# vfmatzkin/ct-unet

Measured on AMD Instinct MI355X. Metric: voxels/sec fwd+bwd, 128^3 fp32 patch, higher is better.
Workload: dtype f32; 1 GPU; UNet() default (1 in, 2 out, i_size 8, 4 blocks), 128^3 patch, batch 1 per GPU, train step = fwd + Dice/CE loss + bwd + grad all-reduce + Adam(amsgrad); patch=128, per_gpu_batch=1, parallelism=dp1, launch=hipgraph

## Files before the change

### ct-unet_amd/csrc/conv3d.hip

```cpp
#include "common.h"
#include "pack.h"
#include "bn_tail.h"
#include "wgrad_reduce.h"

#ifndef CTU_K3S_OCC
#define CTU_K3S_OCC 2
#endif
#ifndef CTU_K3S_ALL
#define CTU_K3S_ALL 1
#endif
#ifndef CTU_WG_OCC
#define CTU_WG_OCC 2
#endif
#ifndef CTU_WG_BLOCKS
#define CTU_WG_BLOCKS 512
#endif

namespace {

typedef float gv2f __attribute__((ext_vector_type(2)));

struct ConvP {
    const float* in;
    const float* in_scale;
// ... 978 lines not shown
__global__ void pack_batch_kernel(PackTable tb) {
    const ctu_pack_job& q = tb.j[blockIdx.y];
    const int idx = blockIdx.x * blockDim.x + threadIdx.x;
    if (q.kind == 1) {
        const int n16 = (q.nout_p + 15) / 16;
        pack_convt_w_elem(idx, q.w, q.wp, q.Ci, q.Co, q.cinv, q.rin_p, n16 <= 1 ? 1 : (n16 <= 2 ? 2 : (n16 <= 4 ? 4 : 8)), q.mode);
    } else if (q.layout == 1) {
        if (q.k == 3) pack_conv_w_pair8_elem<3>(idx, q.w, q.wp, q.Co, q.Ci, q.cinv, q.rin_p / 8, q.mode);
        else pack_conv_w_pair8_elem<5>(idx, q.w, q.wp, q.Co, q.Ci, q.cinv, q.rin_p / 8, q.mode);
    } else if (q.k == 3) {
        pack_conv_w_elem<3>(idx, q.w, q.wp, q.Co, q.Ci, q.cinv, q.rin_p / 8, (q.nout_p + 15) / 16, q.mode);
    } else {
        pack_conv_w_elem<5>(idx, q.w, q.wp, q.Co, q.Ci, q.cinv, q.rin_p / 8, (q.nout_p + 15) / 16, q.mode);
    }
}



template <int KS>
__global__ void pack_conv_w_kernel(const float* __restrict__ w, float* __restrict__ wp, int Co, int Ci,
                                   const int32_t* __restrict__ cinv, int nchunk, int n16, int mode) {
    pack_conv_w_elem<KS>(blockIdx.x * blockDim.x + threadIdx.x, w, wp, Co, Ci, cinv, nchunk, n16, mode);
}

inline void pick_launch(int N, int D, int H, int W, int k, int nout_p, int* nt, int* td, int* th, int* tw) {
    const int n16 = (nout_p + 15) / 16;
    *nt = n16 == 1 ? 1 : (n16 == 2 ? 2 : 4);
    pick_tile(W, td, th, tw);
    auto blocks = [&](int nt_, int td_, int th_, int tw_) {
        return (long)N * ceil_div(D, td_) * ceil_div(H, th_) * ceil_div(W, tw_) * ceil_div(n16, nt_);
    };
    if (*tw == 16 && *nt > 2) *nt = 2;
    while (blocks(*nt, *td, *th, *tw) < 256 && *nt > 1) *nt >>= 1;
    if (blocks(*nt, *td, *th, *tw) < 256 && *tw > 4) { *td = 4; *th = 4; *tw = 4; }
}

struct WgP {
    const float* in;
    const float* in_scale;
    const float* in_shift;
    const float* g;
    float* ws;
    int in_cs, cin_p, in_relu, g_cs, cout_p;
    int N, D, H, W;
    int tiles_d, tiles_h, tiles_w, ntiles;
    int n_ci_t, n_co_t;
    const float* lz_y;
    float* lz_out;
    const float* lz_scale;
    const float* lz_shift;
    const float* lz_coef;
    int lz_cp;
};

template <int KS, int KDS, int TD, int TH, int TW>
__global__ __launch_bounds__(256, CTU_WG_OCC) void conv3d_wgrad_kernel(WgP p) {
    constexpr int PAD = (KS - 1) / 2;
    constexpr int HD = TD + KDS - 1, HH = TH + KS - 1, HW = TW + KS - 1;
    constexpr int HV = HD * HH * HW;
    constexpr int NVOX = TD * TH * TW;
    constexpr int BT = KDS * KS * KS;
    constexpr int KSTEPS = NVOX / 4;
    constexpr int KPW = KSTEPS / 4;
    static_assert(TW % 4 == 0 && KSTEPS % 4 == 0, "tile shape");

    __shared__ __attribute__((aligned(16))) float sA[HV * 16];
    __shared__ __attribute__((aligned(16))) float sG[NVOX * 16];

    const int tid = threadIdx.x, lane = tid & 63, wave = tid >> 6;
    const int i = lane & 15, kq = lane >> 4;
    const int cit = blockIdx.y % p.n_ci_t, cot = blockIdx.y / p.n_ci_t;
    const int kd0 = blockIdx.z * KDS;
    const int ci0 = cit * 16, co0 = cot * 16;

    f32x4 acc[BT];
#pragma unroll
    for (int t = 0; t < BT; ++t) acc[t] = f32x4{0.f, 0.f, 0.f, 0.f};

    const int quad = tid & 3;
    const bool a_ok = (ci0 + quad * 4) < p.cin_p, g_ok = (co0 + quad * 4) < p.cout_p;
    const bool has_xf = p.in_scale != nullptr;
    float4 sc = make_float4(1.f, 1.f, 1.f, 1.f), sh = make_float4(0.f, 0.f, 0.f, 0.f);
    if (has_xf && a_ok) {
        sc = *reinterpret_cast<const float4*>(p.in_scale + ci0 + quad * 4);
        sh = *reinterpret_cast<const float4*>(p.in_shift + ci0 + quad * 4);
    }

    for (int tile = blockIdx.x; tile < p.ntiles; tile += gridDim.x) {
        int bx = tile;
        const int tx = bx % p.tiles_w; bx /= p.tiles_w;
        const int ty = bx % p.tiles_h; bx /= p.tiles_h;
        const int tz = bx % p.tiles_d; bx /= p.tiles_d;
        const int n_img = bx;
        const int d0 = tz * TD, h0 = ty * TH, w0 = tx * TW;
        __syncthreads();
        constexpr int SB = 8;
        const size_t img = (size_t)n_img * p.D * p.H * p.W;
        for (int it0 = tid; it0 < HV * 4; it0 += SB * 256) {
            f32x4 vv[SB];
            unsigned okm = 0;
#pragma unroll
            for (int q = 0; q < SB; ++q) {
                const int it = it0 + q * 256;
                const int v = (it < HV * 4 ? it : it0) >> 2;
                const int pw = v % HW, t2 = v / HW, ph = t2 % HH, pd = t2 / HH;
                const int gd = d0 + pd + kd0 - PAD, gh = h0 + ph - PAD, gw = w0 + pw - PAD;
// ... 56 lines not shown
    for (int t0 = 0; t0 < BT; t0 += RT) {
        __syncthreads();
#pragma unroll
        for (int t = 0; t < BT; ++t)
            if (t >= t0 && t < t0 + RT) {
#pragma unroll
                for (int r = 0; r < 4; ++r) sA[(wave * RT + (t - t0)) * 256 + (kq * 4 + r) * 16 + i] = acc[t][r];
            }
        __syncthreads();
        const int nt = (BT - t0) < RT ? (BT - t0) : RT;
        for (int e = tid; e < nt * 256; e += 256)
            dst[t0 * 256 + e] = (sA[e] + sA[RT * 256 + e]) + (sA[2 * RT * 256 + e] + sA[3 * RT * 256 + e]);
    }
}

template <int KS, int KDS>
__global__ __launch_bounds__(1024) void conv3d_wgrad_reduce_kernel(const float* __restrict__ ws, float* __restrict__ dw,
                                                                  int Co, int Ci, const int32_t* __restrict__ pmap,
                                                                  int cin_p, int n_ci_t, int gx) {
    constexpr int TAPS = KS * KS * KS, BT = KDS * KS * KS;
    __shared__ float red[RPARTS][64];
    const int e = threadIdx.x & 63, part = threadIdx.x >> 6;
    const int el = blockIdx.x * 64 + e;
    const int pz = blockIdx.y;
    float s = 0.f;
    if (el < BT * 256) {
        const float* src = ws + (size_t)pz * gx * (BT * 256) + el;
        for (int k = part; k < gx; k += RPARTS) s += src[(size_t)k * (BT * 256)];
    }
    red[part][e] = s;
    __syncthreads();
    if (part == 0 && el < BT * 256) {
        const float tot = red_total(red, e);
        const int n_pairs = gridDim.y / (TAPS / BT);
        const int z = pz / n_pairs, pair = pz % n_pairs;
        const int cit = pair % n_ci_t, cot = pair / n_ci_t;
        const int tl = el >> 8, i = (el >> 4) & 15, j = el & 15;
        const int cip = cit * 16 + i, co = cot * 16 + j;
        const int ci = (cip < cin_p) ? (pmap ? pmap[cip] : (cip < Ci ? cip : -1)) : -1;
        if (ci >= 0 && co < Co) dw[((size_t)co * Ci + ci) * TAPS + z * BT + tl] = tot;
    }
}

inline bool use_k3s(int k, int W, int cin_p, int cout_p) { return k == 3 && W >= 16 && (CTU_K3S_ALL || cin_p == 8 || cout_p == 8); }

inline int wgrad_gx(int ntiles, int pairs_z) {
    int gx = CTU_WG_BLOCKS / pairs_z;
    if (gx < 1) gx = 1;
    if (gx > ntiles) gx = ntiles;
    return gx;
}


template <int SM, int SN, int UP = 0, bool LZ = false>
__global__ __launch_bounds__(256, CTU_K3S_OCC) void conv3d_wgrad_k3s_kernel(WgP p, int tiles_per_block) {
    static_assert(!UP || (SM == 1 && SN == 1), "the fused up-convolution uses the full 16 x 16 channel tile");
    constexpr int TD = 4, TH = 4, TW = (SM == 2 && SN == 2) ? 16 : 8, HD = 6, HH = 6, HW = TW + 2, HV = HD * HH * HW;
    constexpr int KPR = TW / 4, NKS = TH * KPR;
    constexpr int CM = 16 / SM, CN = 16 / SN;
    constexpr int GW = TW + (SN - 1), GV = TD * TH * GW;
    constexpr int QN = (SM == 2 && SN == 2) ? 1 : ((SM == 1 && SN == 1) ? 3 : 2);
    constexpr int NMF = UP == 2 ? 12 : (UP ? 8 : 9 * QN);
    constexpr int AQ = CM / 4, GQ = CN / 4;
    constexpr int AITEMS = HV * AQ, AITER = (AITEMS + 255) / 256;
    constexpr int GITEMS = GV * GQ, GITER = (GITEMS + 255) / 256;

    constexpr int SAF = AITER * 256 * 4, SGF = GITER * 256 * 4;
    static_assert(SAF >= HV * CM && SGF >= GV * CN, "stage size");
    __shared__ __attribute__((aligned(16))) float sA[2 * SAF];
    __shared__ __attribute__((aligned(16))) float sG[2 * SGF];

    const int tid = threadIdx.x, lane = tid & 63, wave = tid >> 6;
    const int i = lane & 15, kq = lane >> 4;
    const int cig = blockIdx.y % p.n_ci_t, cog = UP ? (blockIdx.y / p.n_ci_t) % p.n_co_t : blockIdx.y / p.n_ci_t;
    const int par = UP ? blockIdx.y / (p.n_ci_t * p.n_co_t) : 0;
    const int pz = UP == 2 ? (par >> 1) & 1 : (par >> 2) & 1, py = UP == 2 ? par & 1 : (par >> 1) & 1, px = UP == 2 ? 0 : par & 1;
    const int gH = UP ? 2 * p.H : p.H, gW = UP ? 2 * p.W : p.W, gs = UP ? 2 : 1;
    const int ci0 = cig * CM, co0 = cog * CN;
    const bool has_xf = p.in_scale != nullptr;

    f32x4 acc[NMF];
#pragma unroll
    for (int t = 0; t < NMF; ++t) acc[t] = f32x4{0.f, 0.f, 0.f, 0.f};

    const int aq = tid % AQ, gq = tid % GQ;
    const bool a_ok = (ci0 + aq * 4) < p.cin_p, g_ok = (co0 + gq * 4) < p.cout_p;
    float4 sc = make_float4(1.f, 1.f, 1.f, 1.f), sh = make_float4(0.f, 0.f, 0.f, 0.f);
    if (has_xf && a_ok) {
        sc = *reinterpret_cast<const float4*>(p.in_scale + ci0 + aq * 4);
        sh = *reinterpret_cast<const float4*>(p.in_shift + ci0 + aq * 4);
    }
    const int xf_relu = has_xf ? p.in_relu : 0;
    const int boff = (SN == 2) ? ((i < 8) ? i : i - 16) : i;

    int tile = blockIdx.x * tiles_per_block;
    const int tile_end = min(p.ntiles, tile + tiles_per_block);
    float4 va[AITER], vg[GITER];
    float4 vy[LZ ? GITER : 1];
    float4 l_sc = make_float4(0.f, 0.f, 0.f, 0.f), l_sh = l_sc, l_k0 = l_sc, l_A = l_sc, l_B = l_sc;
    if constexpr (LZ) {
        const int lzc = (co0 + ((UP && !g_ok) ? 0 : gq * 4)) % p.lz_cp;
        l_sc = *reinterpret_cast<const float4*>(p.lz_scale + lzc);
        l_sh = *reinterpret_cast<const float4*>(p.lz_shift + lzc);
        l_k0 = *reinterpret_cast<const float4*>(p.lz_coef + lzc);
        l_A = *reinterpret_cast<const float4*>(p.lz_coef + 3 * p.lz_cp + lzc);
        l_B = *reinterpret_cast<const float4*>(p.lz_coef + 4 * p.lz_cp + lzc);
    }
    const long long lz_ydelta = LZ ? reinterpret_cast<const char*>(p.lz_y) - reinterpret_cast<const char*>(p.g) : 0;
    const long long lz_odelta = LZ ? reinterpret_cast<const char*>(p.lz_out) - reinterpret_cast<const char*>(p.g) : 0;

    unsigned aoff[AITER], goff[GITER];
    constexpr int FPW = 5;
    unsigned fw[(AITER + FPW - 1) / FPW], gw0 = 0;
#pragma unroll
    for (int q = 0; q < (AITER + FPW - 1) / FPW; ++q) fw[q] = 0;
#pragma unroll
    for (int it = 0; it < AITER; ++it) {
        const int e = tid + it * 256, v = (e < AITEMS) ? e / AQ : 0;
        const int pw = v % HW, t2 = v / HW, ph = t2 % HH, pd = t2 / HH;
        aoff[it] = (unsigned)(((pd * p.H + ph) * p.W + pw) * p.in_cs + ci0 + aq * 4) * 4u;
        const unsigned face = (pd == 0 ? 1u : 0u) | (pd == HD - 1 ? 2u : 0u) | (ph == 0 ? 4u : 0u) | (ph == HH - 1 ? 8u : 0u) |
                              (pw == 0 ? 16u : 0u) | (pw == HW - 1 ? 32u : 0u);
        fw[it / FPW] |= face << (6 * (it % FPW));
    }
#pragma unroll
    for (int it = 0; it < GITER; ++it) {
        const int e = tid + it * 256, v = (e < GITEMS) ? e / GQ : 0;
        const int tw = v % GW, th = (v / GW) % TH, td = v / (GW * TH);
        goff[it] = (unsigned)(((gs * td * gH + gs * th) * gW + gs * tw) * p.g_cs + co0 + gq * 4) * 4u;
        if (SN == 2 && tw == 0) gw0 |= 1u << it;
    }
    const unsigned safe_a = (unsigned)(((p.H + 1) * p.W + 1) * p.in_cs + ci0 + ((UP && !a_ok) ? 0 : aq * 4)) * 4u;
    const unsigned safe_g = (unsigned)((SN - 1) * p.g_cs + co0 + ((UP && !g_ok) ? 0 : gq * 4)) * 4u;
    const bool ch_full = UP || (ci0 + CM <= p.cin_p && co0 + CN <= p.cout_p);

    struct Box { int tx, ty, tz, n; };
    Box box;
    {
        int t = tile;
        box.tx = t % p.tiles_w; t /= p.tiles_w;
        box.ty = t % p.tiles_h; t /= p.tiles_h;
        box.tz = t % p.tiles_d; box.n = t / p.tiles_d;
    }
    auto box_next = [&](Box b) {
        if (++b.tx == p.tiles_w) { b.tx = 0; if (++b.ty == p.tiles_h) { b.ty = 0; if (++b.tz == p.tiles_d) { b.tz = 0; ++b.n; } } }
        return b;
    };

    unsigned amask = 0, gmask = 0;
    const char* pf_abase = nullptr;
    const char* pf_gbase = nullptr;
    unsigned pf_bface = 0;
    auto prep = [&](Box b) -> bool {
        const int d0 = b.tz * TD, h0 = b.ty * TH, w0 = b.tx * TW;
        const long long org = (((long long)b.n * p.D + d0) * p.H + h0) * p.W + w0;
        pf_abase = reinterpret_cast<const char*>(p.in + (org - ((long long)p.H * p.W + p.W + 1)) * p.in_cs);
        if (UP) {
            const long long gorg = (((long long)b.n * 2 * p.D + 2 * d0 + pz) * gH + 2 * h0 + py) * gW + 2 * w0 + px;
            pf_gbase = reinterpret_cast<const char*>(p.g + gorg * p.g_cs);
        } else {
            pf_gbase = reinterpret_cast<const char*>(p.g + (org - (SN - 1)) * p.g_cs);
        }
        pf_bface = (d0 == 0 ? 1u : 0u) | (d0 + TD == p.D ? 2u : 0u) | (h0 == 0 ? 4u : 0u) | (h0 + TH == p.H ? 8u : 0u) |
                   (w0 == 0 ? 16u : 0u) | (w0 + TW == p.W ? 32u : 0u);
        amask = 0; gmask = 0;
        return ch_full && d0 + TD <= p.D && h0 + TH <= p.H && w0 + TW <= p.W;
    };
    auto fetch_a = [&](int it) {
        const bool ok = (fw[it / FPW] & (pf_bface << (6 * (it % FPW)))) == 0u && (!UP || a_ok);
        va[it] = *reinterpret_cast<const float4*>(pf_abase + (ok ? aoff[it] : safe_a));
        amask |= ok ? (1u << it) : 0u;
    };
    auto fetch_g = [&](int it) {
        const bool ok = !((pf_bface & 16u) && ((gw0 >> it) & 1u)) && (!UP || g_ok);
        const unsigned off = ok ? goff[it] : safe_g;
        vg[it] = *reinterpret_cast<const float4*>(pf_gbase + off);
        if constexpr (LZ) vy[it] = *reinterpret_cast<const float4*>(pf_gbase + lz_ydelta + off);
        gmask |= ok ? (1u << it) : 0u;
    };
    auto load_ragged = [&](Box b) {
        const int d0 = b.tz * TD, h0 = b.ty * TH, w0 = b.tx * TW;
#pragma unroll
        for (int it = 0; it < AITER; ++it) {
            const int e = tid + it * 256, v = e / AQ;
            const int pw = v % HW, t2 = v / HW, ph = t2 % HH, pd = t2 / HH;
            const int gd = d0 + pd - 1, gh = h0 + ph - 1, gw = w0 + pw - 1;
            const bool ok = e < AITEMS && a_ok && (unsigned)gd < (unsigned)p.D && (unsigned)gh < (unsigned)p.H &&
                            (unsigned)gw < (unsigned)p.W;
            float4 val = make_float4(0.f, 0.f, 0.f, 0.f);
            if (ok) {
                val = *reinterpret_cast<const float4*>(pf_abase + aoff[it]);
                amask |= 1u << it;
            }
            va[it] = val;
        }
#pragma unroll
        for (int it = 0; it < GITER; ++it) {
            const int e = tid + it * 256, v = e / GQ;
            const int tw = v % GW, th = (v / GW) % TH, td = v / (GW * TH);
            const int gd = d0 + td, gh = h0 + th, gw = w0 + tw - (SN - 1);
            const bool ok = e < GITEMS && g_ok && gd < p.D && gh < p.H && (unsigned)gw < (unsigned)p.W;
            float4 val = make_float4(0.f, 0.f, 0.f, 0.f);
            if (ok) {
                val = *reinterpret_cast<const float4*>(pf_gbase + goff[it]);
                gmask |= 1u << it;
            }
            vg[it] = val;
        }
    };
// ... 850 lines not shown
                                         int in_relu, const float* ga, int g_cs, int cout_p, const float* y,
                                         const float* bn_scale, const float* bn_shift, const float* coef, float* gy_out,
                                         float* dw, int Co, int Ci, const int32_t* cinv, float* ws, int N, int D, int H, int W,
                                         int k, ctu_wgrad_job* job, void* stream) {
    CTU_REQUIRE(job, "conv3d_wgrad_bn_slabs: null job");
    return conv3d_wgrad_bn_impl(in, in_cs, cin_p, in_scale, in_shift, in_relu, ga, g_cs, cout_p, y, bn_scale, bn_shift, coef,
                                gy_out, dw, Co, Ci, cinv, ws, N, D, H, W, k, job, stream);
}

static int conv3d_wgrad_impl(const float* in, int in_cs, int cin_p, const float* in_scale, const float* in_shift,
                             int in_relu, const float* gout, int g_cs, int cout_p, float* dw, float* dbias, int Co,
                             int Ci, const int32_t* cinv, float* ws, int N, int D, int H, int W, int k, const LazyBn* lz,
                             ctu_wgrad_job* job, void* stream) {
    CTU_REQUIRE(k == 3 || k == 5, "conv3d_wgrad: k=%d unsupported (3 or 5)", k);
    CTU_REQUIRE(in && gout && dw && ws, "conv3d_wgrad: null pointer");
    CTU_REQUIRE(cin_p % 8 == 0 && cout_p % 8 == 0 && cin_p > 0 && cout_p > 0, "conv3d_wgrad: padded channels");
    CTU_REQUIRE(in_cs >= cin_p && in_cs % 4 == 0 && g_cs >= cout_p && g_cs % 4 == 0, "conv3d_wgrad: bad stride");
    CTU_REQUIRE(Co <= cout_p && Co > 0 && Ci > 0 && cin_p <= 256, "conv3d_wgrad: Co/Ci");
    CTU_REQUIRE(((uintptr_t)in & 15) == 0 && ((uintptr_t)gout & 15) == 0, "conv3d_wgrad: 16-byte alignment");
    hipStream_t st = (hipStream_t)stream;
    WgP p;
    p.in = in; p.in_scale = in_scale; p.in_shift = in_shift; p.g = gout; p.ws = ws;
    p.in_cs = in_cs; p.cin_p = cin_p; p.in_relu = in_relu; p.g_cs = g_cs; p.cout_p = cout_p;
    p.N = N; p.D = D; p.H = H; p.W = W;
    p.lz_y = nullptr; p.lz_out = nullptr; p.lz_scale = nullptr; p.lz_shift = nullptr; p.lz_coef = nullptr; p.lz_cp = 0;
    if (lz) { p.lz_y = lz->y; p.lz_out = lz->out; p.lz_scale = lz->scale; p.lz_shift = lz->shift; p.lz_coef = lz->coef; p.lz_cp = lz->cp; }
    const WgPlan r = wgrad_plan(N, D, H, W, k, cin_p, cout_p);
    p.tiles_d = r.tiles_d; p.tiles_h = r.tiles_h; p.tiles_w = r.tiles_w;
    p.ntiles = r.ntiles; p.n_ci_t = r.n_ci_g; p.n_co_t = r.n_co_t;
    int rc;
    if (job) *job = ctu_wgrad_job{};
    if (dbias) job = nullptr;
    if (r.kind == WG_K3S) {
        if (r.sm == 2 && r.sn == 2) rc = launch_wgrad_k3s<2, 2>(p, r, dw, Co, Ci, cinv, st, job);
        else if (r.sn == 2) rc = launch_wgrad_k3s<1, 2>(p, r, dw, Co, Ci, cinv, st, job);
        else if (r.sm == 2) rc = launch_wgrad_k3s<2, 1>(p, r, dw, Co, Ci, cinv, st, job);
        else rc = launch_wgrad_k3s<1, 1>(p, r, dw, Co, Ci, cinv, st, job);
    } else if (r.kind == WG_K5S) {
        CTU_REQUIRE((int64_t)((4 + 2 * 2) * H + 8) * W * in_cs * 4 < (int64_t)1 << 31, "conv3d_wgrad: volume too large for 32-bit offsets");
        if (r.sm == 2 && r.sn == 2) rc = launch_wgrad_k5s<2, 2>(p, r, dw, Co, Ci, cinv, st);
        else if (r.sn == 2) rc = launch_wgrad_k5s<1, 2>(p, r, dw, Co, Ci, cinv, st);
        else rc = launch_wgrad_k5s<2, 1>(p, r, dw, Co, Ci, cinv, st);
    } else rc = (k == 3) ? launch_wgrad<3, 3>(p, r, dw, Co, Ci, cinv, st) : launch_wgrad<5, 1>(p, r, dw, Co, Ci, cinv, st);
    if (rc != CTU_OK) return rc;
    if (dbias) return ctu_channel_sum(gout, g_cs, cout_p, (int64_t)N * D * H * W, ws, dbias, Co, stream);
    return CTU_OK;
}

extern "C" size_t ctu_upconv_fused_wgrad_ws_floats(int N, int D, int H, int W, int cin_p, int nout_p) {
    const size_t na = upwg_plan(N, D, H, W, cin_p, nout_p, false).slabs, nb = upwg_plan(N, D, H, W, cin_p, nout_p, true).slabs;
    return na > nb ? na : nb;
}

static int upconv_fused_wgrad_impl(const float* in, int in_cs, int cin_p, const float* in_scale, const float* in_shift,
                                   int in_relu, const float* gout, int g_cs, int nout_p, float* dweff, float* ws,
                                   int N, int D, int H, int W, const LazyBn* lz, void* stream);

extern "C" int ctu_upconv_fused_wgrad(const float* in, int in_cs, int cin_p, const float* in_scale, const float* in_shift,
                                      int in_relu, const float* gout, int g_cs, int nout_p, float* dweff, float* ws,
                                      int N, int D, int H, int W, void* stream) {
    return upconv_fused_wgrad_impl(in, in_cs, cin_p, in_scale, in_shift, in_relu, gout, g_cs, nout_p, dweff, ws, N, D, H, W,
                                   nullptr, stream);
}

extern "C" int ctu_upconv_fused_wgrad_bn_supported(int N, int D, int H, int W, int cin_p, int nout_p) {
    return (N > 0 && D % 4 == 0 && H % 4 == 0 && W % 8 == 0 && cin_p % 16 == 0 && nout_p % 8 == 0) ? 1 : 0;
}

extern "C" int ctu_upconv_fused_wgrad_bn(const float* in, int in_cs, int cin_p, const float* in_scale, const float* in_shift,
                                         int in_relu, const float* ga, int g_cs, int nout_p, const float* y,
                                         const float* bn_scale, const float* bn_shift, const float* coef, float* gy_out,
                                         float* dweff, float* ws, int N, int D, int H, int W, void* stream) {
    CTU_REQUIRE(y && bn_scale && bn_shift && coef && gy_out, "upconv_fused_wgrad_bn: null pointer");
    CTU_REQUIRE(ctu_upconv_fused_wgrad_bn_supported(N, D, H, W, cin_p, nout_p), "upconv_fused_wgrad_bn: geometry not supported");
    CTU_REQUIRE(((uintptr_t)y & 15) == 0 && ((uintptr_t)gy_out & 15) == 0 && gy_out != ga, "upconv_fused_wgrad_bn: y / gy_out alignment, gy_out must not alias ga");
    const LazyBn lz = {y, bn_scale, bn_shift, coef, gy_out, nout_p};
    return upconv_fused_wgrad_impl(in, in_cs, cin_p, in_scale, in_shift, in_relu, ga, g_cs, nout_p, dweff, ws, N, D, H, W, &lz, stream);
}

static int upconv_fused_wgrad_impl(const float* in, int in_cs, int cin_p, const float* in_scale, const float* in_shift,
                                   int in_relu, const float* gout, int g_cs, int nout_p, float* dweff, float* ws,
                                   int N, int D, int H, int W, const LazyBn* lz, void* stream) {
    CTU_REQUIRE(in && gout && dweff && ws, "upconv_fused_wgrad: null pointer");
    CTU_REQUIRE(cin_p % 8 == 0 && nout_p % 8 == 0 && cin_p > 0 && nout_p > 0 && nout_p <= 64, "upconv_fused_wgrad: padded channels");
    CTU_REQUIRE(in_cs >= cin_p && in_cs % 4 == 0 && g_cs >= nout_p && g_cs % 4 == 0, "upconv_fused_wgrad: bad stride");
    CTU_REQUIRE(((uintptr_t)in & 15) == 0 && ((uintptr_t)gout & 15) == 0, "upconv_fused_wgrad: 16-byte alignment");
    CTU_REQUIRE((in_scale == nullptr) == (in_shift == nullptr), "upconv_fused_wgrad: scale/shift must come together");
    CTU_REQUIRE((int64_t)(2 * H * W + 2 * W + 2) * in_cs * 4 < (int64_t)1 << 31 && (int64_t)(8 * 2 * H + 8) * 2 * W * g_cs * 4 < (int64_t)1 << 31,
                "upconv_fused_wgrad: volume too large for 32-bit offsets");
    hipStream_t st = (hipStream_t)stream;
    const bool pw = nout_p == 8 && g_cs == 8;
    const UpWgPlan g = upwg_plan(N, D, H, W, cin_p, nout_p, pw);
    WgP p;
    p.in = in; p.in_scale = in_scale; p.in_shift = in_shift; p.g = gout; p.ws = ws;
    p.in_cs = in_cs; p.cin_p = cin_p; p.in_relu = in_relu; p.g_cs = g_cs; p.cout_p = nout_p;
    p.N = N; p.D = D; p.H = H; p.W = W;
    p.tiles_d = ceil_div(D, 4); p.tiles_h = ceil_div(H, 4); p.tiles_w = ceil_div(W, 8);
    p.ntiles = g.ntiles; p.n_ci_t = g.n_ci_g; p.n_co_t = g.n_co_g;
    p.lz_y = nullptr; p.lz_out = nullptr; p.lz_scale = nullptr; p.lz_shift = nullptr; p.lz_coef = nullptr; p.lz_cp = 0;
    if (lz) { p.lz_y = lz->y; p.lz_out = lz->out; p.lz_scale = lz->scale; p.lz_shift = lz->shift; p.lz_coef = lz->coef; p.lz_cp = lz->cp; }
    if (pw) {
        p.cout_p = 16;
        if (lz) conv3d_wgrad_k3s_kernel<1, 1, 2, true><<<dim3(g.grid.gx, g.pairs), 256, 0, st>>>(p, g.grid.tpb);
        else conv3d_wgrad_k3s_kernel<1, 1, 2><<<dim3(g.grid.gx, g.pairs), 256, 0, st>>>(p, g.grid.tpb);
        CTU_CHECK_LAUNCH("upconv_fused_wgrad(pw)");
        upconv_wgrad_reduce_pw_kernel<<<dim3(12 * 256 / 64, g.pairs), 64 * RPARTS, 0, st>>>(ws, dweff, cin_p, g.n_ci_g, g.grid.gx);
        CTU_CHECK_LAUNCH("upconv_fused_wgrad_reduce(pw)");
        return CTU_OK;
    }
    if (lz) conv3d_wgrad_k3s_kernel<1, 1, 1, true><<<dim3(g.grid.gx, g.pairs), 256, 0, st>>>(p, g.grid.tpb);
    else conv3d_wgrad_k3s_kernel<1, 1, 1><<<dim3(g.grid.gx, g.pairs), 256, 0, st>>>(p, g.grid.tpb);
    CTU_CHECK_LAUNCH("upconv_fused_wgrad");
    upconv_wgrad_reduce_kernel<<<dim3(8 * 256 / 64, g.pairs), 64 * RPARTS, 0, st>>>(ws, dweff, cin_p, nout_p, g.n_ci_g, g.n_co_g, g.grid.gx);
    CTU_CHECK_LAUNCH("upconv_fused_wgrad_reduce");
    return CTU_OK;
}
```

### ct-unet_amd/csrc/upconv_fused.hip

```cpp
#include <type_traits>
#include "common.h"
#include "bn_tail.h"
#include "channel_sum.h"

namespace {

typedef float v2f __attribute__((ext_vector_type(2)));

struct UpP {
    const float* in;
    const float* in_scale;
    const float* in_shift;
    const float* wp;
    const float* beff;
    float* out;
    float* stats;
    int in_cs, rin_p, in_relu, out_cs, nout_p;
    int N, D, H, W;
    int tiles_d, tiles_h, tiles_w;
    ctu_bn_tail tail;
};

template <int PB, int NTP, bool PW = false>
__global__ __launch_bounds__(256, 2) void upconv_fused_fwd_kernel(UpP p, int ntiles, int tiles_per_block) {
    static_assert(PW ? (PB == 4 && NTP == 1) : ((PB * NTP == 8 || (PB == 4 && NTP == 1)) && (PB == 8 || PB == 4 || PB == 2)), "tile-parities per block");
    constexpr int NTW = PW ? 3 : 2, TAPS = 4 * NTW;
    constexpr int MT = 4, TD = 4, TH = 4, TW = 16;
    constexpr int HD = TD + 2, HH = TH + 2, HW = TW + 2, HV = HD * HH * HW;
    constexpr int NTHR = 256;
    constexpr int NTPT = NTP;
    constexpr int WFL = PB * TAPS * NTP * 128;
    constexpr int AITEMS = HV * 2, AITER = (AITEMS + NTHR - 1) / NTHR;
    constexpr int WITER = (WFL / 4 + NTHR - 1) / NTHR;
    constexpr int VS2 = 6;
    static_assert(WFL / 4 % NTHR == 0, "weight staging covers the stage exactly");

    __shared__ __attribute__((aligned(16))) v2f sA2[HV * VS2];
    __shared__ __attribute__((aligned(16))) v2f sW2[WFL / 2];
    typedef const volatile __attribute__((address_space(3))) v2f* lds_v2f_ptr;
    __shared__ float sRed[4 * NTP * 16 * 2];

    const int tid = threadIdx.x, lane = tid & 63, wave = tid >> 6;
    const int m = lane & 15, kq = lane >> 4;
    const int by = blockIdx.y;
    const int nchunk = p.rin_p >> 3;
    const int half = tid & 1;
    const bool has_xf = p.in_scale != nullptr;
    const int pd0 = PW ? 0 : ((by * PB) >> 2) & 1, ph0 = PW ? 0 : ((by * PB) >> 1) & 1;

    lds_v2f_ptr vA = (lds_v2f_ptr)sA2 + (((wave + pd0) * HH + ph0) * HW + m) * VS2 + kq;
    lds_v2f_ptr vW = (lds_v2f_ptr)sW2 + (kq * 16 + m);

    unsigned hoff[AITER];
    constexpr int FPW = 5, NFW = (AITER + FPW - 1) / FPW;
    unsigned fw[NFW];
#pragma unroll
    for (int q = 0; q < NFW; ++q) fw[q] = 0;
#pragma unroll
    for (int it = 0; it < AITER; ++it) {
        const int i = tid + it * NTHR;
        const int v = (i < AITEMS) ? (i >> 1) : 0;
        const int pw = v % HW, t2 = v / HW, ph = t2 % HH, pd = t2 / HH;
        hoff[it] = (unsigned)(((pd * p.H + ph) * p.W + pw) * p.in_cs + half * 4) * 4u;
        const unsigned face = (pd == 0 ? 1u : 0u) | (pd == HD - 1 ? 2u : 0u) | (ph == 0 ? 4u : 0u) | (ph == HH - 1 ? 8u : 0u) |
                              (pw == 0 ? 16u : 0u) | (pw == HW - 1 ? 32u : 0u);
        fw[it / FPW] |= face << (6 * (it % FPW));
    }
    const unsigned safe_off = (unsigned)(((p.H + 1) * p.W + 1) * p.in_cs + half * 4) * 4u;

    f32x4 acc[PB][MT][NTP];
    float s1[NTP][4], s2[NTP][4];
#pragma unroll
    for (int nt = 0; nt < NTP; ++nt) {
#pragma unroll
        for (int pi = 0; pi < PB; ++pi)
#pragma unroll
            for (int mt = 0; mt < MT; ++mt) acc[pi][mt][nt] = f32x4{0.f, 0.f, 0.f, 0.f};
#pragma unroll
        for (int r = 0; r < 4; ++r) { s1[nt][r] = 0.f; s2[nt][r] = 0.f; }
    }

    int tile = blockIdx.x * tiles_per_block;
    const int tile_end = min(ntiles, tile + tiles_per_block);
    int c = 0;
    float4 va[AITER];
    typedef typename std::conditional<PW, f32x4, float4>::type wv_t;
    wv_t vw[WITER];
    float4 sc = make_float4(1.f, 1.f, 1.f, 1.f), sh = make_float4(0.f, 0.f, 0.f, 0.f);
    unsigned vmask = 0;

    struct Box { int tx, ty, tz, n; };
    Box box;
    {
        int t = tile;
        box.tx = t % p.tiles_w; t /= p.tiles_w;
        box.ty = t % p.tiles_h; t /= p.tiles_h;
        box.tz = t % p.tiles_d; box.n = t / p.tiles_d;
    }
    auto box_next = [&](Box b) {
        if (++b.tx == p.tiles_w) { b.tx = 0; if (++b.ty == p.tiles_h) { b.ty = 0; if (++b.tz == p.tiles_d) { b.tz = 0; ++b.n; } } }
        return b;
    };
    bool a_interior = false;
    auto load_a = [&](Box b, int cc) {
        const int d0 = b.tz * TD, h0 = b.ty * TH, w0 = b.tx * TW;
        if (has_xf) {
            sc = *reinterpret_cast<const float4*>(p.in_scale + cc * 8 + half * 4);
            sh = *reinterpret_cast<const float4*>(p.in_shift + cc * 8 + half * 4);
        }
        const long long org = (((long long)b.n * p.D + d0) * p.H + h0) * p.W + w0 - ((long long)p.H * p.W + p.W + 1);
        const char* base = reinterpret_cast<const char*>(p.in + org * p.in_cs + cc * 8);
        a_interior = d0 >= 1 && h0 >= 1 && w0 >= 1 && d0 + TD < p.D && h0 + TH < p.H && w0 + TW < p.W;
        if (a_interior) {
#pragma unroll
            for (int it = 0; it < AITER; ++it) {
                if ((it + 1) * NTHR <= AITEMS || tid + it * NTHR < AITEMS)
                    va[it] = *reinterpret_cast<const float4*>(base + hoff[it]);
                else
                    va[it] = make_float4(0.f, 0.f, 0.f, 0.f);
            }
            return;
        }
        vmask = 0;
        if (d0 + TD <= p.D && h0 + TH <= p.H && w0 + TW <= p.W) {
            const unsigned bface = (d0 == 0 ? 1u : 0u) | (d0 + TD == p.D ? 2u : 0u) | (h0 == 0 ? 4u : 0u) |
                                   (h0 + TH == p.H ? 8u : 0u) | (w0 == 0 ? 16u : 0u) | (w0 + TW == p.W ? 32u : 0u);
#pragma unroll
            for (int it = 0; it < AITER; ++it) {
                const bool ok = (fw[it / FPW] & (bface << (6 * (it % FPW)))) == 0u;
                va[it] = *reinterpret_cast<const float4*>(base + (ok ? hoff[it] : safe_off));
                vmask |= ok ? (1u << it) : 0u;
            }
            return;
        }
#pragma unroll
        for (int it = 0; it < AITER; ++it) {
            const int i = tid + it * NTHR, v = i >> 1;
            const int pw = v % HW, t2 = v / HW, ph = t2 % HH, pd = t2 / HH;
            const int gd = d0 + pd - 1, gh = h0 + ph - 1, gw = w0 + pw - 1;
            const bool ok = i < AITEMS && (unsigned)gd < (unsigned)p.D && (unsigned)gh < (unsigned)p.H && (unsigned)gw < (unsigned)p.W;
            float4 val = make_float4(0.f, 0.f, 0.f, 0.f);
            if (ok) {
                val = *reinterpret_cast<const float4*>(base + hoff[it]);
                vmask |= 1u << it;
            }
            va[it] = val;
        }
    };
    auto load_w = [&](int cc) {
        const char* wsrc = reinterpret_cast<const char*>(PW ? p.wp + (size_t)cc * 4 * TAPS * 128
                                                            : p.wp + ((size_t)cc * 8 + (size_t)by * PB) * 8 * NTPT * 128);
#pragma unroll
        for (int it = 0; it < WITER; ++it) vw[it] = *reinterpret_cast<const wv_t*>(wsrc + (unsigned)(tid + it * NTHR) * 16u);
    };
    if (tile >= tile_end) return;
    load_a(box, 0);
    load_w(0);

    while (true) {
        CTU_SETPRIO(CTU_PRIO_STAGE);
        __syncthreads();
        {
            auto put = [&](int it, float4 val) {
                const int i = tid + it * NTHR;
// ... 102 lines not shown
                            *reinterpret_cast<float4*>(p.out + fv * p.out_cs + co) = o;
                            s1[nt][0] += o.x; s1[nt][1] += o.y; s1[nt][2] += o.z; s1[nt][3] += o.w;
                            s2[nt][0] += o.x * o.x; s2[nt][1] += o.y * o.y; s2[nt][2] += o.z * o.z; s2[nt][3] += o.w * o.w;
                        }
                        acc[pi][mt][nt] = f32x4{0.f, 0.f, 0.f, 0.f};
                    }
                }
            }
        }
        if (!has_next) break;
        tile = ntile; c = nc; box = nbox;
    }
    if (p.stats) {
        __syncthreads();
#pragma unroll
        for (int nt = 0; nt < NTP; ++nt)
#pragma unroll
            for (int r = 0; r < 4; ++r) {
                float a1 = s1[nt][r], a2 = s2[nt][r];
#pragma unroll
                for (int o = 1; o < 16; o <<= 1) { a1 += __shfl_xor(a1, o); a2 += __shfl_xor(a2, o); }
                if (PW) { a1 += __shfl_xor(a1, 32); a2 += __shfl_xor(a2, 32); }
                const int ch = PW ? (kq & 1) * 4 + r : nt * 16 + kq * 4 + r;
                if (m == 0 && (!PW || kq < 2)) {
                    sRed[(wave * NTP * 16 + ch) * 2 + 0] = a1;
                    sRed[(wave * NTP * 16 + ch) * 2 + 1] = a2;
                }
            }
        __syncthreads();
        float* row = p.stats + ((size_t)blockIdx.y * gridDim.x + blockIdx.x) * 2 * p.nout_p;
        for (int ch = tid; ch < p.nout_p; ch += NTHR) {
            float a1 = 0.f, a2 = 0.f;
#pragma unroll
            for (int w = 0; w < 4; ++w) {
                a1 += sRed[(w * NTP * 16 + ch) * 2 + 0];
                a2 += sRed[(w * NTP * 16 + ch) * 2 + 1];
            }
            st_row(p.tail.counter != nullptr, row + ch, a1);
            st_row(p.tail.counter != nullptr, row + p.nout_p + ch, a2);
        }
        if (p.tail.counter) bn_fwd_tail(p.tail, p.stats, gridDim.x * gridDim.y, p.nout_p, gridDim.x * gridDim.y);
    }
}

struct UpDP {
    const float* g;
    const float* wp;
    float* out;
    int g_cs, nout_p, out_cs, cin_p;
    int N, D, H, W;
    int tiles_d, tiles_h, tiles_w, n16;
};

template <int NT>
__global__ __launch_bounds__(256, 2) void upconv_fused_bwd_data_kernel(UpDP p, int ntiles, int tiles_per_block) {
    constexpr int MT = 4, TD = 4, TH = 4, TW = 16;
    constexpr int HD = TD + 2, HH = TH + 2, HW = TW + 2, HV = HD * HH * HW;
    constexpr int NTHR = 256;
    constexpr int WFL = 8 * NT * 128;
    constexpr int AITEMS = HV * 2, AITER = (AITEMS + NTHR - 1) / NTHR;
    constexpr int WITER = (WFL / 4 + NTHR - 1) / NTHR;
    constexpr int VS2 = 6;
    static_assert(WFL / 4 % NTHR == 0, "weight staging covers the stage exactly");

    __shared__ __attribute__((aligned(16))) v2f sA2[HV * VS2];
    __shared__ __attribute__((aligned(16))) v2f sW2[WFL / 2];
    typedef const volatile __attribute__((address_space(3))) v2f* lds_v2f_ptr;

    const int tid = threadIdx.x, lane = tid & 63, wave = tid >> 6;
    const int m = lane & 15, kq = lane >> 4;
    const int by = blockIdx.y;
    const int qc = p.nout_p >> 3;
    const int nchunk = 8 * qc;
    const int half = tid & 1;
    const int Hf = 2 * p.H, Wf = 2 * p.W;

    lds_v2f_ptr vA0 = (lds_v2f_ptr)sA2 + ((wave * HH) * HW + m) * VS2 + kq;
    lds_v2f_ptr vW = (lds_v2f_ptr)sW2 + (kq * 16 + m);

    unsigned hoff[AITER];
    constexpr int FPW = 5, NFW = (AITER + FPW - 1) / FPW;
    unsigned fw[NFW];
#pragma unroll
    for (int q = 0; q < NFW; ++q) fw[q] = 0;
#pragma unroll
    for (int it = 0; it < AITER; ++it) {
        const int i = tid + it * NTHR;
        const int v = (i < AITEMS) ? (i >> 1) : 0;
        const int pw = v % HW, t2 = v / HW, ph = t2 % HH, pd = t2 / HH;
        hoff[it] = (unsigned)(((2 * pd * Hf + 2 * ph) * Wf + 2 * pw) * p.g_cs + half * 4) * 4u;
        const unsigned face = (pd == 0 ? 1u : 0u) | (pd == HD - 1 ? 2u : 0u) | (ph == 0 ? 4u : 0u) | (ph == HH - 1 ? 8u : 0u) |
                              (pw == 0 ? 16u : 0u) | (pw == HW - 1 ? 32u : 0u);
        fw[it / FPW] |= face << (6 * (it % FPW));
    }
    const unsigned safe_off = (unsigned)(((2 * Hf + 2) * Wf + 2) * p.g_cs + half * 4) * 4u;

    f32x4 acc[MT][NT];
#pragma unroll
    for (int nt = 0; nt < NT; ++nt)
#pragma unroll
        for (int mt = 0; mt < MT; ++mt) acc[mt][nt] = f32x4{0.f, 0.f, 0.f, 0.f};

    int tile = blockIdx.x * tiles_per_block;
    const int tile_end = min(ntiles, tile + tiles_per_block);
    if (tile >= tile_end) return;
    int c = 0;
    float4 va[AITER], vw[WITER];
    unsigned vmask = 0;
// ... 99 lines not shown
        if (nc == nchunk) { nc = 0; ntile = tile + 1; nbox = box_next(box); }
        const bool has_next = ntile < tile_end;
        if (has_next) {
            load_a(nbox, nc);
            load_w(nc);
        }
        CTU_SETPRIO(0);
        {
            v2f ar[2][5], br[2][2][NT];
            auto load_group = [&](int g, v2f (&aa)[5], v2f (&bb)[2][NT]) {
                const int ez = (g >> 1) & 1, ex = g & 1;
#pragma unroll
                for (int r = 0; r < 5; ++r) aa[r] = vA[((ez * HH + r) * HW + ex) * VS2];
#pragma unroll
                for (int ey = 0; ey < 2; ++ey)
#pragma unroll
                    for (int nt = 0; nt < NT; ++nt) bb[ey][nt] = vW[(((ez * 2 + ey) * 2 + ex) * NT + nt) * 64];
            };
            load_group(0, ar[0], br[0]);
#if CTU_PIN_FWD
            __builtin_amdgcn_sched_barrier(0);
#endif
#pragma unroll
            for (int g = 0; g < 4; ++g) {
                if (g + 1 < 4) load_group(g + 1, ar[(g + 1) & 1], br[(g + 1) & 1]);
                v2f (&aa)[5] = ar[g & 1];
                v2f (&bb)[2][NT] = br[g & 1];
#pragma unroll
                for (int ey = 0; ey < 2; ++ey) {
#pragma unroll
                    for (int nt = 0; nt < NT; ++nt)
#pragma unroll
                        for (int mt = 0; mt < MT; ++mt)
                            acc[mt][nt] = __builtin_amdgcn_mfma_f32_16x16x4f32(bb[ey][nt].x, aa[mt + ey].x, acc[mt][nt], 0, 0, 0);
#pragma unroll
                    for (int nt = 0; nt < NT; ++nt)
#pragma unroll
                        for (int mt = 0; mt < MT; ++mt)
                            acc[mt][nt] = __builtin_amdgcn_mfma_f32_16x16x4f32(bb[ey][nt].y, aa[mt + ey].y, acc[mt][nt], 0, 0, 0);
                }
#if CTU_PIN_FWD
#pragma unroll
                for (int q = 0; q < 4 * MT * NT; ++q) {
                    __builtin_amdgcn_sched_group_barrier(0x008, 1, 0);
                    if (g + 1 < 4 && q < 5 + 2 * NT) __builtin_amdgcn_sched_group_barrier(0x100, 1, 0);
                }
#endif
            }
        }
        CTU_SETPRIO(CTU_PRIO_STAGE);
        if (c == nchunk - 1) {
            const int d0 = box.tz * TD, h0 = box.ty * TH, w0 = box.tx * TW;
            const int gw = w0 + m;
            float* obase = p.out + ((((size_t)box.n * p.D + d0 + wave) * p.H + h0) * p.W + gw) * p.out_cs;
            const int orow = p.W * p.out_cs;
#pragma unroll
            for (int nt = 0; nt < NT; ++nt) {
                const int co = (by * NT + nt) * 16 + kq * 4;
#pragma unroll
                for (int mt = 0; mt < MT; ++mt) {
                    if (co < p.cin_p && d0 + wave < p.D && h0 + mt < p.H && gw < p.W) {
                        float4 o;
                        o.x = acc[mt][nt][0]; o.y = acc[mt][nt][1]; o.z = acc[mt][nt][2]; o.w = acc[mt][nt][3];
                        *reinterpret_cast<float4*>(obase + mt * orow + co) = o;
                    }
                    acc[mt][nt] = f32x4{0.f, 0.f, 0.f, 0.f};
                }
            }
        }
        if (!has_next) break;
        tile = ntile; c = nc; box = nbox;
    }
}

__device__ __forceinline__ float upconv_pack_bwd_value(const float* __restrict__ wp, int idx, int cin_p, int nout_p) {
    const int n16 = (cin_p + 15) >> 4, qc = nout_p >> 3, ntpt = (nout_p + 15) >> 4;
    int r = idx;
    const int j = r & 1; r >>= 1;
    const int n = r & 15; r >>= 4;
    const int kq = r & 3; r >>= 2;
    const int nt = r % n16; r /= n16;
    const int e = r & 7; r >>= 3;
    const int q = r % qc;
    const int par = r / qc;
    const int pos = nt * 16 + n, co = q * 8 + kq * 2 + j;
    float v = 0.f;
    if (pos < cin_p) {
        const int cf = pos >> 3, kqf = (pos & 7) >> 1, jf = pos & 1;
        v = wp[((((size_t)cf * 8 + par) * 8 + (e ^ 7)) * ntpt + (co >> 4)) * 128 + kqf * 32 + (co & 15) * 2 + jf];
    }
    return v;
}

__device__ __forceinline__ int axis_pairs(int pbit, int jbit, int (&t)[2], int (&a)[2]) {
    if (pbit == 0) {
        if (jbit == 0) { t[0] = 0; a[0] = 1; return 1; }
        t[0] = 1; a[0] = 0; t[1] = 2; a[1] = 1; return 2;
    }
    if (jbit == 0) { t[0] = 0; a[0] = 0; t[1] = 1; a[1] = 1; return 2; }
    t[0] = 2; a[0] = 0; return 1;
}

__global__ void upconv_transpose_kernel(const float* __restrict__ wt, const float* __restrict__ w3, float* __restrict__ wtt,
                                        float* __restrict__ w3t, int C, int Co, int nout_p) {
    const int idx = blockIdx.x * blockDim.x + threadIdx.x;
    const int n3 = 27 * C * nout_p, nt = 8 * C * C;
    if (idx < n3) {
        const int co = idx % nout_p, cm = (idx / nout_p) % C, t = idx / (nout_p * C);
        w3t[idx] = co < Co ? w3[((size_t)co * C + cm) * 27 + t] : 0.f;
    } else if (idx < n3 + nt) {
        const int k = idx - n3;
        const int cm = k % C, ci = (k / C) % C, a = k / (C * C);
        wtt[k] = wt[((size_t)ci * C + cm) * 8 + a];
    }
}

constexpr int WS_WAVES = 8, WS_BLOCK = WS_WAVES * 64;
// ... 306 lines not shown
}

extern "C" int ctu_upconv_fused_supported(int k, int D, int H, int W, int cin_p, int nout_p) {
    return k == 3 && W >= 16 && D >= 1 && H >= 1 && cin_p % 8 == 0 && cin_p >= 8 && nout_p % 8 == 0 && nout_p >= 8 && nout_p <= 64;
}

static size_t up_std_packed(int cin_p, int nout_p) { return (size_t)(cin_p / 8) * 8 * 8 * ceil_div(nout_p, 16) * 128; }

extern "C" size_t ctu_upconv_fused_packed_floats(int cin_p, int nout_p) {
    return up_std_packed(cin_p, nout_p) + (nout_p == 8 ? (size_t)(cin_p / 8) * 4 * 12 * 128 : 0);
}

extern "C" int ctu_upconv_fused_num_blocks(int N, int D, int H, int W, int nout_p) {
    const UpPlan r = up_plan(N, D, H, W, nout_p, 0);
    return r.grid.gx * r.ny;
}

extern "C" size_t ctu_upconv_fused_pack_ws_floats(int C, int nout_p) { return (size_t)27 * C * nout_p + (size_t)8 * C * C; }

static int upconv_pack_gather(const float* wp, int cin_p, int nout_p, float* wpw, float* wpd, hipStream_t st) {
    const int npw = wpw ? (cin_p / 8) * 4 * 12 * 128 : 0;
    const int nwpd = wpd ? (int)ctu_upconv_fused_bwd_packed_floats(cin_p, nout_p) : 0;
    if (npw + nwpd == 0) return CTU_OK;
    upconv_pack_gather_kernel<<<ceil_div(npw + nwpd, 256), 256, 0, st>>>(wp, wpw, npw, wpd, nwpd, cin_p, nout_p);
    CTU_CHECK_LAUNCH("upconv_fused_pack_gather");
    return CTU_OK;
}

extern "C" int ctu_upconv_fused_pack_all(const float* wt, const float* bt, const float* w3, int C, int Co, const int32_t* cinv,
                                         int cin_p, int nout_p, float* wp, float* beff, float* ws, float* wpd, void* stream) {
    CTU_REQUIRE(wt && bt && w3 && wp && beff && ws, "upconv_fused_pack: null pointer");
    CTU_REQUIRE(C > 0 && Co > 0 && Co <= nout_p && cin_p % 8 == 0 && nout_p % 8 == 0 && (cinv || C <= cin_p),
                "upconv_fused_pack: C=%d Co=%d cin_p=%d nout_p=%d", C, Co, cin_p, nout_p);
    hipStream_t st = (hipStream_t)stream;
    const int ntpt = ceil_div(nout_p, 16);
    CTU_REQUIRE(((uintptr_t)ws & 15) == 0, "upconv_fused_pack: ws must be 16-byte aligned");
    float* w3t = ws;
    float* wtt = ws + (size_t)27 * C * nout_p;
    const int ntr = 27 * C * nout_p + 8 * C * C;
    upconv_transpose_kernel<<<ceil_div(ntr, 256), 256, 0, st>>>(wt, w3, wtt, w3t, C, Co, nout_p);
    CTU_CHECK_LAUNCH("upconv_fused_transpose");
    const int quads = (cin_p / 8) * 8 * 8 * 8 * ntpt * 4;
    upconv_pack_beff_kernel<<<nout_p / BEFF_CO + ceil_div(quads, 8), WS_BLOCK, 0, st>>>(wtt, w3t, wp, C, nout_p, cinv, cin_p / 8,
                                                                                         ntpt, bt, beff);
    CTU_CHECK_LAUNCH("upconv_fused_pack");
    return upconv_pack_gather(wp, cin_p, nout_p, nout_p == 8 ? wp + up_std_packed(cin_p, nout_p) : nullptr, wpd, st);
}

extern "C" int ctu_upconv_fused_pack(const float* wt, const float* bt, const float* w3, int C, int Co, const int32_t* cinv,
                                     int cin_p, int nout_p, float* wp, float* beff, float* ws, void* stream) {
    return ctu_upconv_fused_pack_all(wt, bt, w3, C, Co, cinv, cin_p, nout_p, wp, beff, ws, nullptr, stream);
}

extern "C" int ctu_upconv_fused_fwd(const float* in, int in_cs, int cin_p, const float* in_scale, const float* in_shift,
                                    int in_relu, const float* wp, const float* beff, float* out, int out_cs, int nout_p,
                                    float* stats, int N, int D, int H, int W, const ctu_bn_tail* tail, void* stream) {
    CTU_REQUIRE(in && wp && beff && out, "upconv_fused_fwd: null pointer");
    CTU_REQUIRE(ctu_upconv_fused_supported(3, D, H, W, cin_p, nout_p), "upconv_fused_fwd: unsupported geometry (W=%d cin_p=%d nout_p=%d)",
                W, cin_p, nout_p);
    CTU_REQUIRE(in_cs >= cin_p && in_cs % 4 == 0 && out_cs >= nout_p && out_cs % 4 == 0, "upconv_fused_fwd: bad stride");
    CTU_REQUIRE((in_scale == nullptr) == (in_shift == nullptr), "upconv_fused_fwd: scale/shift must come together");
    CTU_REQUIRE(((uintptr_t)in & 15) == 0 && ((uintptr_t)out & 15) == 0 && ((uintptr_t)wp & 15) == 0 && ((uintptr_t)beff & 15) == 0,
                "upconv_fused_fwd: 16-byte alignment");
    CTU_REQUIRE((int64_t)N * D * H * W * 8 < (int64_t)1 << 31 && (int64_t)(2 * H * W + 2 * W + 2) * in_cs * 4 < (int64_t)1 << 31,
                "upconv_fused_fwd: volume too large for 32-bit offsets");
    UpP p;
    p.in = in; p.in_scale = in_scale; p.in_shift = in_shift; p.wp = wp; p.beff = beff; p.out = out; p.stats = stats;
    CTU_REQUIRE(!tail || (stats && tail->counter && tail->gamma && tail->beta && tail->scale && tail->shift && tail->mean &&
                          tail->invstd && tail->C > 0 && tail->C <= nout_p && tail->count > 0),
                "upconv_fused_fwd: incomplete BatchNorm tail");
    p.tail = tail_or_off(tail);
    p.in_cs = in_cs; p.rin_p = cin_p; p.in_relu = in_relu; p.out_cs = out_cs; p.nout_p = nout_p;
    p.N = N; p.D = D; p.H = H; p.W = W;
    const UpPlan r = up_plan(N, D, H, W, nout_p, 0);
    p.tiles_d = r.tiles_d; p.tiles_h = r.tiles_h; p.tiles_w = r.tiles_w;
    const int ny = r.ny, gx = r.grid.gx, tpb = r.grid.tpb, ntiles = r.ntiles;
    hipStream_t st = (hipStream_t)stream;
    if (nout_p == 16 && ny == 2) {
        upconv_fused_fwd_kernel<4, 1><<<dim3(gx, 2), 256, 0, st>>>(p, ntiles, tpb);
    } else if (nout_p == 8) {
        p.wp = wp + up_std_packed(cin_p, nout_p);
        upconv_fused_fwd_kernel<4, 1, true><<<dim3(gx, 1), 256, 0, st>>>(p, ntiles, tpb);
    } else if (ny == 1) upconv_fused_fwd_kernel<8, 1><<<dim3(gx, 1), 256, 0, st>>>(p, ntiles, tpb);
    else if (ny == 2) upconv_fused_fwd_kernel<4, 2><<<dim3(gx, 2), 256, 0, st>>>(p, ntiles, tpb);
    else upconv_fused_fwd_kernel<2, 4><<<dim3(gx, 4), 256, 0, st>>>(p, ntiles, tpb);
    CTU_CHECK_LAUNCH("upconv_fused_fwd");
    return CTU_OK;
}

extern "C" int ctu_channel_sum_num_blocks(int64_t nvox);

extern "C" size_t ctu_upconv_fused_project_ws_floats(int nout_p, int64_t fine_nvox) {
    return (size_t)27 * FS_SPLIT * nout_p + (size_t)27 * nout_p + nout_p + (size_t)ctu_channel_sum_num_blocks(fine_nvox) * nout_p;
}

static int upconv_project_impl(int dtype, const float* dweff, const void* gout, int g_cs, int nout_p, int N, int D, int H, int W,
                               const float* bt, const float* pack_ws, const int32_t* imap, int C, int Co, int cin_p,
                               float* dwt, float* dbt, float* dw3, float* ws, void* stream) {
    CTU_REQUIRE(dweff && gout && bt && pack_ws && dwt && dbt && dw3 && ws, "upconv_fused_project: null pointer");
    CTU_REQUIRE(nout_p == 8 || nout_p == 16 || nout_p == 32 || nout_p == 64, "upconv_fused_project: nout_p=%d", nout_p);
    CTU_REQUIRE(C > 0 && Co > 0 && Co <= nout_p && g_cs >= nout_p && g_cs % 4 == 0, "upconv_fused_project: bad channels");
    CTU_REQUIRE(((uintptr_t)dweff & 15) == 0 && ((uintptr_t)pack_ws & 15) == 0, "upconv_fused_project: dweff / pack_ws must be 16-byte aligned");
    hipStream_t st = (hipStream_t)stream;
    float* tpart = ws;
    float* V = ws + (size_t)27 * FS_SPLIT * nout_p;
    float* tall = V + (size_t)27 * nout_p;
    float* csp = tall + nout_p;
    const int64_t fvox = (int64_t)N * 8 * D * H * W;
    const int nb = ctu_channel_sum_num_blocks(fvox);
    const int nsum = nb + 26 * FS_SPLIT;
    if (dtype == 0) {
        upconv_sums_kernel<float><<<nsum, 256, 0, st>>>((const float*)gout, g_cs, nout_p, N, 2 * D, 2 * H, 2 * W, fvox, csp, nb, tpart);
    } else {
        CTU_DISPATCH_LP(dtype, upconv_sums_kernel<T><<<nsum, 256, 0, st>>>((const T*)gout, g_cs, nout_p, N, 2 * D, 2 * H, 2 * W, fvox, csp, nb, tpart));
    }
    CTU_CHECK_LAUNCH("upconv_sums");
    upconv_tall_v_kernel<<<nout_p, 256, 0, st>>>(csp, nb, tpart, nout_p, tall, V);
    CTU_CHECK_LAUNCH("upconv_tall_v");
    const float* w3t = pack_ws;
    const float* wtt = pack_ws + (size_t)27 * C * nout_p;
    const int nb1 = ceil_div((C * C * 8 + C) * 8, WS_BLOCK);
    const int nb2 = ceil_div(((Co + 3) / 4) * C * 27, 8);
    upconv_project_kernel<<<nb1 + nb2, WS_BLOCK, 0, st>>>(dweff, V, wtt, w3t, bt, imap, C, Co, cin_p, nout_p, nb1, dwt, dw3, dbt);
    CTU_CHECK_LAUNCH("upconv_project");
    return CTU_OK;
}

extern "C" int ctu_upconv_fused_project(const float* dweff, const float* gout, int g_cs, int nout_p, int N, int D, int H, int W,
                                        const float* bt, const float* pack_ws, const int32_t* imap, int C, int Co, int cin_p,
                                        float* dwt, float* dbt, float* dw3, float* ws, void* stream) {
    return upconv_project_impl(0, dweff, gout, g_cs, nout_p, N, D, H, W, bt, pack_ws, imap, C, Co, cin_p, dwt, dbt, dw3, ws, stream);
}
extern "C" int ctu_lp_upconv_fused_project(int dtype, const float* dweff, const void* gout, int g_cs, int nout_p, int N, int D, int H,
                                           int W, const float* bt, const float* pack_ws, const int32_t* imap, int C, int Co, int cin_p,
                                           float* dwt, float* dbt, float* dw3, float* ws, void* stream) {
    CTU_REQUIRE(dtype == CTU_BF16 || dtype == CTU_F16, "lp_upconv_fused_project: dtype %d", dtype);
    return upconv_project_impl(dtype, dweff, gout, g_cs, nout_p, N, D, H, W, bt, pack_ws, imap, C, Co, cin_p, dwt, dbt, dw3, ws, stream);
}

extern "C" size_t ctu_upconv_fused_bwd_packed_floats(int cin_p, int nout_p) {
    return (size_t)8 * (nout_p / 8) * 8 * ceil_div(cin_p, 16) * 128;
}

extern "C" int ctu_upconv_fused_pack_bwd(const float* wp, int cin_p, int nout_p, float* wpd, void* stream) {
    CTU_REQUIRE(wp && wpd && cin_p % 8 == 0 && nout_p % 8 == 0, "upconv_fused_pack_bwd: bad argument");
    return upconv_pack_gather(wp, cin_p, nout_p, nullptr, wpd, (hipStream_t)stream);
}

extern "C" int ctu_upconv_fused_bwd_data(const float* gout, int g_cs, int nout_p, const float* wpd, float* gin, int gin_cs,
                                         int cin_p, int N, int D, int H, int W, void* stream) {
    CTU_REQUIRE(gout && wpd && gin, "upconv_fused_bwd_data: null pointer");
    CTU_REQUIRE(ctu_upconv_fused_supported(3, D, H, W, cin_p, nout_p), "upconv_fused_bwd_data: unsupported geometry");
    CTU_REQUIRE(g_cs >= nout_p && g_cs % 4 == 0 && gin_cs >= cin_p && gin_cs % 4 == 0, "upconv_fused_bwd_data: bad stride");
    CTU_REQUIRE(((uintptr_t)gout & 15) == 0 && ((uintptr_t)gin & 15) == 0 && ((uintptr_t)wpd & 15) == 0, "upconv_fused_bwd_data: alignment");
    CTU_REQUIRE((int64_t)(12 * 2 * H + 12) * 2 * W * g_cs * 4 + 64 < (int64_t)1 << 31, "upconv_fused_bwd_data: volume too large for 32-bit offsets");
    UpDP p;
    p.g = gout; p.wp = wpd; p.out = gin; p.g_cs = g_cs; p.nout_p = nout_p; p.out_cs = gin_cs; p.cin_p = cin_p;
    p.N = N; p.D = D; p.H = H; p.W = W;
    p.n16 = ceil_div(cin_p, 16);
    const UpPlan r = up_plan(N, D, H, W, nout_p, p.n16);
    p.tiles_d = r.tiles_d; p.tiles_h = r.tiles_h; p.tiles_w = r.tiles_w;
    const int NT = r.nt, ny = r.ny, gx = r.grid.gx, tpb = r.grid.tpb, ntiles = r.ntiles;
    hipStream_t st = (hipStream_t)stream;
    if (NT == 4) upconv_fused_bwd_data_kernel<4><<<dim3(gx, ny), 256, 0, st>>>(p, ntiles, tpb);
    else if (NT == 2) upconv_fused_bwd_data_kernel<2><<<dim3(gx, ny), 256, 0, st>>>(p, ntiles, tpb);
    else upconv_fused_bwd_data_kernel<1><<<dim3(gx, ny), 256, 0, st>>>(p, ntiles, tpb);
    CTU_CHECK_LAUNCH("upconv_fused_bwd_data");
    return CTU_OK;
}
```

### ct-unet_amd/ctunet_amd/_lib.py

```python
from __future__ import annotations

import ctypes as C
import os

import torch

_HERE = os.path.dirname(os.path.abspath(__file__))
LIB_PATH = os.environ.get("CTUNET_HIP_LIB") or os.path.join(_HERE, "libctunet_hip.so")

P = C.c_void_p
I = C.c_int
L = C.c_int64
F = C.c_float
D = C.c_double
Z = C.c_size_t
U = C.c_uint64

class PackJob(C.Structure):
    _fields_ = [("w", C.c_void_p), ("wp", C.c_void_p), ("cinv", C.c_void_p), ("kind", C.c_int), ("Co", C.c_int),
                ("Ci", C.c_int), ("k", C.c_int), ("rin_p", C.c_int), ("nout_p", C.c_int), ("mode", C.c_int),
                ("layout", C.c_int)]


class BnTail(C.Structure):
# ... 54 lines not shown
    "ctu_bn_bwd_num_blocks": (I, [L]),
    "ctu_bn_relu_bwd_reduce": (I, [P, I, P, I, I, P, P, P, P, L, P, P, P]),
    "ctu_bn_bwd_finalize": (I, [P, I, I, I, D, P, P, P, P, P, P, P, P, F, F, P, P]),
    "ctu_bn_relu_bwd_apply": (I, [P, I, P, I, I, P, P, P, P, P, L, P]),
    "ctu_conv3d_wgrad_slabs": (I, [P, I, I, P, P, I, P, I, I, P, P, I, I, P, P, I, I, I, I, I, P, P]),
    "ctu_conv3d_wgrad_bn_slabs": (I, [P, I, I, P, P, I, P, I, I, P, P, P, P, P, P, I, I, P, P, I, I, I, I, I, P, P]),
    "ctu_conv3d_first_wgrad_slabs": (I, [P, I, P, I, P, I, P, I, I, I, I, P, P]),
    "ctu_conv3d_first_wgrad_bn_slabs": (I, [P, I, P, I, P, P, P, P, P, P, I, P, I, I, I, I, P, P]),
    "ctu_convt2_wgrad_slabs": (I, [P, I, I, P, P, I, P, I, I, P, P, I, I, P, P, I, I, I, I, P, P]),
    "ctu_bn_bwd_finalize_jobs": (I, [P, I, I, I, D, P, P, P, P, P, P, P, P, F, F, P, P, I, P]),
    "ctu_wgrad_reduce_jobs": (I, [P, I, P]),
    "ctu_maxpool2_fwd": (I, [P, I, I, P, P, I, P, I, I, I, I, I, P]),
    "ctu_maxpool2_bwd": (I, [P, I, I, P, P, I, P, I, P, I, I, I, I, I, I, P]),
    "ctu_maxpool2_bwd_bn_num_blocks": (I, [I, I, I, I, I]),
    "ctu_maxpool2_bwd_bn": (I, [P, I, I, P, P, P, P, P, I, P, I, I, I, I, I, I, P, P, P]),
    "ctu_convt_packed_floats": (Z, [I, I]),
    "ctu_pack_convt_weight": (I, [P, P, I, I, P, I, I, I, P]),
    "ctu_convt2_fwd": (I, [P, I, I, P, P, I, P, P, I, P, I, I, I, I, I, I, P]),
    "ctu_convt2_bwd_data": (I, [P, I, I, P, P, I, I, I, I, I, I, P]),
    "ctu_convt2_wgrad_ws_floats": (Z, [I, I, I, I, I, I]),
    "ctu_convt2_wgrad": (I, [P, I, I, P, P, I, P, I, I, P, P, I, I, P, P, I, I, I, I, P]),
    "ctu_convt2_plan": (C.c_char_p, [I, I, I, I, I, I, I, P]),
    "ctu_convt2_wgrad_plan": (C.c_char_p, [I, I, I, I, I, I, P]),
    "ctu_head_fwd": (I, [P, I, I, P, P, I, P, P, P, I, I, I, I, P, P, I, L, P]),
    "ctu_head_bwd_ws_floats": (Z, [I, L, I, I]),
    "ctu_head_bwd": (I, [P, I, I, P, P, I, P, P, P, I, I, I, I, P, P, P, I, P, P, P, I, L, P]),
    "ctu_head_bwd_num_blocks": (I, [I, L]),
    "ctu_head_bwd_bn": (I, [P, I, I, P, P, I, P, P, P, I, I, I, I, P, P, P, I, P, P, P, I, L, P, P, I, P, P, P]),
    "ctu_head_fwd_seg2": (I, [P, I, P, I, I, P, P, I, P, P, P, I, I, I, I, P, P, I, L, P]),
    "ctu_head_bwd_bn_seg2": (I, [P, I, P, I, I, P, P, I, P, P, P, I, I, I, I, P, P, P, I, P, I, P, P, P, I, L, P, P, I, P, P, P]),
    "ctu_loss_ws_floats": (Z, [I, L]),
    "ctu_loss_fwd": (I, [P, P, I, L, F, F, I, P, P, P]),
    "ctu_loss_bwd": (I, [P, P, I, L, F, F, I, P, P, P, P, I, P]),
    "ctu_seg_loss_ws_floats": (Z, [I, L]),
    "ctu_seg_loss_fwd": (I, [P, P, P, I, L, P, P, P, P]),
    "ctu_seg_loss_bwd": (I, [P, P, P, I, L, P, P, P, P, P, P, P, I, P]),
    "ctu_skip_add": (I, [P, I, P, P, I, P, I, P, P, I, P, I, I, L, P]),
    "ctu_upconv_fused_supported": (I, [I, I, I, I, I, I]),
    "ctu_upconv_fused_packed_floats": (Z, [I, I]),
    "ctu_upconv_fused_num_blocks": (I, [I, I, I, I, I]),
    "ctu_upconv_fused_pack_ws_floats": (Z, [I, I]),
    "ctu_upconv_fused_pack": (I, [P, P, P, I, I, P, I, I, P, P, P, P]),
    "ctu_upconv_fused_pack_all": (I, [P, P, P, I, I, P, I, I, P, P, P, P, P]),
    "ctu_upconv_fused_fwd": (I, [P, I, I, P, P, I, P, P, P, I, I, P, I, I, I, I, P, P]),
    "ctu_upconv_fused_wgrad_ws_floats": (Z, [I, I, I, I, I, I]),
    "ctu_upconv_fused_wgrad": (I, [P, I, I, P, P, I, P, I, I, P, P, I, I, I, I, P]),
    "ctu_upconv_fused_wgrad_bn_supported": (I, [I, I, I, I, I, I]),
    "ctu_upconv_fused_wgrad_bn": (I, [P, I, I, P, P, I, P, I, I, P, P, P, P, P, P, P, I, I, I, I, P]),
    "ctu_upconv_fused_project_ws_floats": (Z, [I, L]),
    "ctu_upconv_fused_project": (I, [P, P, I, I, I, I, I, I, P, P, P, I, I, I, P, P, P, P, P]),
    "ctu_upconv_fused_bwd_packed_floats": (Z, [I, I]),
    "ctu_upconv_fused_pack_bwd": (I, [P, I, I, P, P]),
    "ctu_upconv_fused_bwd_data": (I, [P, I, I, P, P, I, I, I, I, I, I, P]),
    "ctu_hard_segm": (I, [P, I, I, L, P, P]),
    "ctu_one_hot": (I, [P, I, I, L, P, P]),
    "ctu_hard_dice_ws_doubles": (Z, [I]),
    "ctu_hard_dice_counts": (I, [P, P, I, I, L, P, P, P]),
    "ctu_hausdorff_ws_bytes": (Z, [I, I, I, I, I]),
    "ctu_hausdorff": (I, [P, P, I, I, I, I, I, P, P, P]),
    "ctu_surface_ws_bytes": (Z, [I, I, I, I, I]),
    "ctu_surface_metrics": (I, [P, I, I, P, I, I, I, I, I, I, I, I, I, P, P, D, P, P, P]),
    "ctu_components_ws_bytes": (Z, [I, I, I, I]),
    "ctu_label_components": (I, [P, I, I, I, I, I, I, P, I, P, P, P, P]),
    "ctu_filter_components": (I, [P, I, I, I, I, I, I, P, I, I, I, P, P, P]),
    "ctu_morphology_ws_bytes": (Z, [I, I, I, I, I]),
    "ctu_binary_morphology": (I, [P, I, I, I, I, I, I, C.c_uint32, I, I, I, L, P, P, P]),
    "ctu_fill_holes": (I, [P, I, I, I, I, I, I, I, L, P, P, P]),
    "ctu_implant_mask": (I, [P, I, P, I, I, I, I, I, C.c_uint32, I, I, I, I, P, P, P]),
    "ctu_distance_ws_bytes": (Z, [I, I, I, I, I, I]),
    "ctu_distance_transform": (I, [P, I, I, I, I, I, I, L, I, I, P, I, P, P, F, P, P]),
    "ctu_thickness_ws_bytes": (Z, [I, I, I, I, I]),
    "ctu_local_thickness": (I, [P, I, I, I, I, I, P, P, P, P]),
    "ctu_thickness_summary_ws_bytes": (Z, [I, L]),
    "ctu_thickness_summary": (I, [P, I, L, F, P, P, P]),
    "ctu_resample": (I, [P, I, I, I, L, I, I, I, I, I, I, P, P, P, P, P]),
    "ctu_affine_resample": (I, [P, I, I, I, L, I, I, I, I, I, I, P, P, P, P, P, D, P, P]),
    "ctu_registration_ws_bytes": (Z, [L]),
    "ctu_registration_init": (I, [P, L, P, P, P]),
    "ctu_registration_accumulate": (I, [P, L, P, I, I, I, P, P, D, P, P]),
    "ctu_registration_update": (I, [L, I, P, P, P, I, P, P]),
    "ctu_similarity_ws_bytes": (Z, [L, L]),
    "ctu_similarity_init": (I, [P, L, P, P, P]),
    "ctu_similarity_accumulate": (I, [I, P, L, P, I, I, I, P, P, P, L, P, I, I, I, P, P, D, P, P]),
    "ctu_similarity_update": (I, [I, L, L, I, P, P, P, I, P, P]),
    "ctu_ffd_ws_bytes": (Z, [P, L]),
    "ctu_ffd_cells": (I, [P, L, P, P, P, P, P, P]),
    "ctu_ffd_init": (I, [P, L, P, D, P, P, P]),
    "ctu_ffd_accumulate": (I, [P, L, P, P, I, I, I, P, P, P, P, P, D, P, P, P, P, L, P, P]),
    "ctu_ffd_update": (I, [L, P, P, P, P, L, I, P, P, I, P, P]),
    "ctu_ffd_transform_points": (I, [P, L, P, P, P, P, P, P, P, P]),
    "ctu_ffd_resample": (I, [P, I, I, I, L, I, I, I, I, I, I, P, P, P, P, P, P, P, P, P, D, P, P]),
    "ctu_mesh_ws_bytes": (Z, [I, I, I]),
    "ctu_mesh_count": (I, [P, I, I, I, I, I, L, F, P, P]),
    "ctu_mesh_emit": (I, [P, I, I, I, I, F, F, P, P, L, L, P, P, P, P]),
    "ctu_mesh_measure": (I, [P, L, P, L, P, P, P, P]),
    "ctu_mesh_adjacency_ws_bytes": (Z, [L, L]),
    "ctu_mesh_adjacency_build": (I, [P, L, L, P, P, P]),
    "ctu_mesh_adjacency_emit": (I, [L, L, L, P, P, P, P]),
    "ctu_mesh_smooth_ws_bytes": (Z, [L]),
    "ctu_mesh_smooth": (I, [P, L, P, P, L, P, I, F, I, F, P, P, P]),
    "ctu_mesh_voxelize_ws_bytes": (Z, [I, I, I]),
    "ctu_mesh_voxelize": (I, [P, L, P, L, I, I, I, P, P, I, P, P, P]),
    "ctu_mesh_grid_ws_bytes": (Z, [L, L]),
    "ctu_mesh_grid_build": (I, [P, L, P, L, F, L, P, P, P]),
    "ctu_mesh_grid_emit": (I, [P, L, L, L, L, P, P, P, P]),
    "ctu_mesh_distance": (I, [P, L, P, P, L, P, I, I, I, P, L, I, I, I, P, P, F, F, P, P, P, P]),
# ... 179 lines not shown
```

### ct-unet_amd/ctunet_amd/engine.py

```python
from __future__ import annotations

import os
from dataclasses import dataclass
from typing import Dict, List, Optional, Tuple

import torch

from . import ops
from .ops import CL, pad8

BN_EPS = 1e-5
FUSE_UP = os.environ.get("CTUNET_FUSE_UP", "1") != "0"
FUSE_UP_MAX_CO = int(os.environ.get("CTUNET_FUSE_UP_MAXCO", "16"))
POOL_BN = os.environ.get("CTUNET_POOL_BN", "1") != "0"
LP_FUSE_UP = os.environ.get("CTUNET_LP_FUSE_UP", "1") != "0"
BN_MOMENTUM = 0.1
LAZY_BN = os.environ.get("CTUNET_LAZY_BN", "1") != "0"
LAZY_BN_LP = os.environ.get("CTUNET_LAZY_BN_LP", "0") != "0"
BN_TAIL = os.environ.get("CTUNET_BN_TAIL", "0") != "0"
DEFER_WGRAD_REDUCE = os.environ.get("CTUNET_DEFER_WGRAD_REDUCE", "1") != "0"
SPLIT_CAT0 = os.environ.get("CTUNET_SPLIT_CAT0", "1") != "0"


def _cat_halves(buf: torch.Tensor, cp: int):
    if buf.dim() == 6:
        return CL(buf[0], 0, cp), CL(buf[1], 0, cp)
    return CL(buf, 0, cp), CL(buf, cp, cp)


@dataclass
class BlockPlan:
    prefix: str
    first: int
    cin: int
    cout: int


@dataclass
class NetPlan:
    k: int
    conv_bias: bool
    in_ch: int
    out_ch: int
    enc: List[BlockPlan]
    center: BlockPlan
    center_live: bool
    dec: List[BlockPlan]
    head: str
    act: int
    head_mode: int
    skip: str = "cat"


@dataclass(slots=True)
class _ConvRec:
    x: Optional[CL]
    y: CL
    vec: torch.Tensor
    stats: Optional[torch.Tensor]
    nblk: int
    conv: str
    bn: str
    cin: int
    cout: int
    imap: Optional[torch.Tensor]
    bias: bool
    first: Optional[torch.Tensor] = None


class _WgradWs:

    def __init__(self, floats: int, device, defer: bool):
        self.jobs = ops.WgradJobs() if defer else None
        self.bufs = [torch.empty(floats, dtype=torch.float32, device=device) for _ in range(2 if defer else 1)]
        self.i = 0

    def take(self) -> torch.Tensor:
        self.i = (self.i + 1) % len(self.bufs)
        ws = self.bufs[self.i]
        if self.jobs is not None:
# ... 89 lines not shown
                continue
            ver = (w._version, w.data_ptr())
            if force or ent[0] != ver:
                jobs.append((kind, w.detach().contiguous(), ent[1], ent[2], rin_p, nout_p, mode, layout))
                self._pack_cache[key] = (ver, ent[1], ent[2])
        ops.pack_batch(jobs, self.dtype)

    def invalidate_packs(self) -> None:
        for key, ent in self._pack_cache.items():
            self._pack_cache[key] = (None,) + tuple(ent[1:])
        for prefix, hit in self._up_cache.items():
            self._up_cache[prefix] = (None,) + tuple(hit[1:])

    def _fwd_tail(self, P, bn: str, c: int, nvox: int, n_upd: int, vec4: torch.Tensor, device):
        counter = self._counter(bn, "fwd", device)
        if counter is None:
            return None
        return ops.make_bn_tail(c, nvox, P[bn + ".weight"], P[bn + ".bias"], P[bn + ".running_mean"], P[bn + ".running_var"],
                                BN_MOMENTUM, BN_EPS, n_upd, vec4, P.get(bn + ".num_batches_tracked") if n_upd else None,
                                counter)

    def _bn_stage(self, P, bn: str, out: CL, vec4: torch.Tensor, nvox: int, c: int, training: bool, n_upd: int, nblk: int,
                  launch, tail_ok: bool = True) -> Tuple[CL, Optional[torch.Tensor]]:
        wb = (P[bn + ".weight"], P[bn + ".bias"], P[bn + ".running_mean"], P[bn + ".running_var"])
        if training:
            stats = torch.empty((nblk, 2, out.cp), dtype=torch.float32, device=out.buf.device)
            tail = self._fwd_tail(P, bn, c, nvox, n_upd, vec4, out.buf.device) if tail_ok else None
            launch(stats, tail)
            if tail is None:
                ops.bn_finalize_into(stats, nblk, c, out.cp, nvox, *wb, BN_MOMENTUM, BN_EPS, n_upd, vec4,
                                     P.get(bn + ".num_batches_tracked") if n_upd else None)
        else:
            stats = None
            launch(None, None)
            ops.bn_eval_affine_into(*wb, BN_EPS, c, out.cp, vec4)
        return out.with_xf(vec4[0], vec4[1], True), stats

    def _conv_bn(self, P, x: CL, conv: str, bn: str, cin: int, cout: int, imap, out: CL, vec4: torch.Tensor,
                 training: bool, n_upd: int, save: bool) -> Tuple[CL, Optional[_ConvRec]]:
        k = self.plan.k
        w = P[conv + ".weight"]
        bias = P.get(conv + ".bias")
        lay = ops.conv_layout(k, out.cp, x.dims[3], self.dtype, x.cp)
        if bias is not None and self.dtype != torch.float32:
            lay = 0
        wp = self._packed(conv, w, "conv", imap, x.cp, out.cp, 0, lay)
        bias_p = None if bias is None else bias.detach()
        nblk = ops.conv_num_blocks(x.dims, out.cp, lay, k, self.dtype, x.cp) if training else 0
        y, stats = self._bn_stage(P, bn, out, vec4, x.nvox, cout, training, n_upd, nblk,
                                  lambda stats, tail: ops.conv3d_fwd(x, wp, bias_p, out, k, stats, (cin, cout), lay, tail))
        rec = _ConvRec(x, out.raw(), vec4, stats, nblk, conv, bn, cin, cout, imap, bias is not None) if save else None
        return y, rec

    def _fuse_up(self, x: CL, nout_p: int) -> bool:
        if not (self.plan.k == 3 and not self.plan.conv_bias and nout_p <= FUSE_UP_MAX_CO and FUSE_UP):
            return False
        if self.dtype == torch.float32:
            return ops.upconv_fused_supported(x.dims, 3, x.cp, nout_p)
        return LP_FUSE_UP and ops.lp_upconv_fused_supported(x.dims, 3, x.cp, nout_p)

    def _upconv_bn(self, P, x: CL, prefix: str, ct: int, cout: int, cinv, out: CL, vec4: torch.Tensor, training: bool,
                   n_upd: int, save: bool) -> Tuple[CL, Optional[_ConvRec]]:
        conv, bn = f"{prefix}.1", f"{prefix}.2"
        wt, bt, w3 = P[f"{prefix}.0.weight"], P[f"{prefix}.0.bias"], P[conv + ".weight"]
        lp = bool(x.lp)
        ver = tuple((t._version, t.data_ptr()) for t in (wt, bt, w3))
        hit = self._up_cache.get(prefix)
        if hit is None or hit[0] != ver or hit[3] != (x.cp, out.cp, self.dtype) or torch.cuda.is_current_stream_capturing():
            same = hit is not None and hit[3] == (x.cp, out.cp, self.dtype)
            if lp:
                wp, beff, pws = ops.upconv_fused_pack(wt, bt, w3, cinv, x.cp, out.cp, (hit[1], hit[2], hit[4]) if same else None)
                wpd = ops.lp_upconv_fused_pack(wp, x.cp, self.dtype, hit[5] if same else None)
            else:
                wp, beff, pws, wpd = ops.upconv_fused_pack_all(wt, bt, w3, cinv, x.cp, out.cp,
                                                               (hit[1], hit[2], hit[4], hit[5]) if same else None)
            self._up_cache[prefix] = (ver, wp, beff, (x.cp, out.cp, self.dtype), pws, wpd)
        else:
            wp, beff, wpd = hit[1], hit[2], hit[5]
        if lp:
            nblk = ops.lp_upconv_fused_num_blocks(x.dims) if training else 0
            launch = lambda stats, tail: ops.lp_upconv_fused_fwd(x, wpd, beff, out, stats, (ct, cout))
        else:
            nblk = ops.upconv_fused_num_blocks(x.dims, out.cp) if training else 0
            launch = lambda stats, tail: ops.upconv_fused_fwd(x, wp, beff, out, stats, (ct, cout), tail)
        y, stats = self._bn_stage(P, bn, out, vec4, 8 * x.nvox, cout, training, n_upd, nblk, launch, tail_ok=not lp)
        rec = _ConvRec(None, out.raw(), vec4, stats, nblk, conv, bn, ct, cout, None, False) if save else None
        return y, rec

    def _first_conv_bn(self, P, x: torch.Tensor, conv: str, bn: str, cin: int, cout: int, out: CL, vec4: torch.Tensor,
                       training: bool, n_upd: int, save: bool):
        w = P[conv + ".weight"].detach()
        bias = P.get(conv + ".bias")
        bias_p = None if bias is None else bias.detach()
        nblk = ops.conv_first_num_blocks(out.dims) if training else 0
        y, stats = self._bn_stage(P, bn, out, vec4, out.nvox, cout, training, n_upd, nblk,
                                  lambda stats, tail: ops.conv_first_fwd(x, w, bias_p, out, stats, tail))
        rec = _ConvRec(None, out.raw(), vec4, stats, nblk, conv, bn, cin, cout, None, bias is not None, x) if save else None
        return y, rec

    def forward(self, P: Dict[str, torch.Tensor], x: torch.Tensor, training: bool, save: bool, chk: bool):
        plan = self.plan
        dev = x.device
        n, cin, d, h, w = x.shape
        nlev = len(plan.enc)
        if cin != plan.in_ch:
            raise RuntimeError(f"ctunet_amd: expected {plan.in_ch} input channels, got {cin}")
        if any(s % (1 << nlev) for s in (d, h, w)):
            raise RuntimeError(f"ctunet_amd: spatial size {(d, h, w)} must be divisible by {1 << nlev}")
        if training and n * (d >> nlev) * (h >> nlev) * (w >> nlev) <= 1:
            raise ValueError("Expected more than 1 value per channel when training (centre block)")
        ctx = {"recs": {}, "levels": [], "training": training, "chk": chk} if save else None
        n_upd = 1 if training else 0
        self.refresh_packs(P)

        x = x.contiguous()
        e0 = plan.enc[0]
        first_direct = plan.conv_bias is False and ops.conv_first_supported(plan.k, cin, pad8(e0.cout), w)
        adt = self.dtype
        cur = None if first_direct else ops.ncdhw_to_cl(x, dtype=adt)
        x_cl = cur
        cat: List[torch.Tensor] = []
        halves = []
        xf: List[torch.Tensor] = []
        pooled: List[CL] = []
        dskip: List[CL] = []
        dd, hh, ww = d, h, w
        recs = {}
        xf_sizes = [8 * pad8(blk.cout) for blk in plan.enc]
        xf_all = torch.zeros(sum(xf_sizes), dtype=torch.float32, device=dev)
        xf_off = 0
        for i, blk in enumerate(plan.enc):
            cp = pad8(blk.cout)
            split = SPLIT_CAT0 and i == 0 and cp <= 16
            cat.append(torch.empty((2, n, dd, hh, ww, cp) if split else (n, dd, hh, ww, 2 * cp), dtype=adt, device=dev))
            halves.append(_cat_halves(cat[i], cp))
            xf.append(xf_all[xf_off:xf_off + 8 * cp].view(4, 2 * cp))
            xf_off += 8 * cp
            t1 = CL(torch.empty((n, dd, hh, ww, cp), dtype=adt, device=dev), 0, cp)
            v1 = torch.empty((4, cp), dtype=torch.float32, device=dev)
            imap = None
            if i == 0 and first_direct:
                a1, recs[(blk.prefix, 1)] = self._first_conv_bn(P, x, f"{blk.prefix}.{blk.first}",
                                                                f"{blk.prefix}.{blk.first + 1}", blk.cin, blk.cout, t1,
                                                                v1, training, n_upd, save)
            else:
                a1, recs[(blk.prefix, 1)] = self._conv_bn(P, cur, f"{blk.prefix}.{blk.first}",
                                                          f"{blk.prefix}.{blk.first + 1}", blk.cin, blk.cout, imap, t1,
                                                          v1, training, n_upd, save)
            a2, recs[(blk.prefix, 2)] = self._conv_bn(P, a1, f"{blk.prefix}.{blk.first + 3}", f"{blk.prefix}.{blk.first + 4}",
                                                      blk.cout, blk.cout, None, halves[i][1], xf[i][:, cp:],
                                                      training, n_upd, save)
            dskip.append(a2)
            dd, hh, ww = dd // 2, hh // 2, ww // 2
            pl = CL(torch.empty((n, dd, hh, ww, cp), dtype=adt, device=dev), 0, cp)
            ops.maxpool_fwd(a2, pl)
            pooled.append(pl)
            cur = pl
        cb = plan.center
        cpc = pad8(cb.cout)
        center_out = None
        if plan.center_live or training:
            live = plan.center_live
            c1 = CL(torch.empty((n, dd, hh, ww, cpc), dtype=adt, device=dev), 0, cpc)
            c2 = CL(torch.empty((n, dd, hh, ww, cpc), dtype=adt, device=dev), 0, cpc)
            v1 = torch.empty((4, cpc), dtype=torch.float32, device=dev)
            v2 = torch.empty((4, cpc), dtype=torch.float32, device=dev)
            a1, r1 = self._conv_bn(P, cur, f"{cb.prefix}.{cb.first}", f"{cb.prefix}.{cb.first + 1}", cb.cin, cb.cout,
                                   None, c1, v1, training, n_upd, save and live)
            a2, r2 = self._conv_bn(P, a1, f"{cb.prefix}.{cb.first + 3}", f"{cb.prefix}.{cb.first + 4}", cb.cout, cb.cout,
                                   None, c2, v2, training, n_upd, save and live)
            if live:
                recs[(cb.prefix, 1)], recs[(cb.prefix, 2)] = r1, r2
                center_out = a2
        cur = center_out if plan.center_live else pooled[-1]
        cur_segs = ((cb.cout if plan.center_live else plan.enc[-1].cout, 0),)
        dec_in: List[CL] = []
        ups: List[CL] = []
        for j, blk in enumerate(plan.dec):
            i = nlev - 1 - j
            cp = pad8(blk.cout)
            dd, hh, ww = dd * 2, hh * 2, ww * 2
            ct = blk.cin
            ctp = pad8(ct)
            imap_t, cinv_t = self._maps(cur_segs, cur.cp, dev)
            wt = P[f"{blk.prefix}.0.weight"]
            dec_in.append(cur)
            t1 = CL(torch.empty((n, dd, hh, ww, cp), dtype=adt, device=dev), 0, cp)
            v1 = torch.empty((4, cp), dtype=torch.float32, device=dev)
            if self._fuse_up(cur, cp):
                ups.append(None)
                a1, recs[(blk.prefix, 1)] = self._upconv_bn(P, cur, blk.prefix, ct, blk.cout, cinv_t, t1, v1, training,
                                                            n_upd, save)
            else:
                up = CL(torch.empty((n, dd, hh, ww, ctp), dtype=adt, device=dev), 0, ctp)
                wpt = self._packed(f"{blk.prefix}.0", wt, "convt", cinv_t, cur.cp, ctp, 0)
                ops.convt_fwd(cur, wpt, P[f"{blk.prefix}.0.bias"].detach(), up)
                ups.append(up)
                a1, recs[(blk.prefix, 1)] = self._conv_bn(P, up, f"{blk.prefix}.1", f"{blk.prefix}.2", ct, blk.cout, None,
                                                          t1, v1, training, n_upd, save)
            a2, recs[(blk.prefix, 2)] = self._conv_bn(P, a1, f"{blk.prefix}.4", f"{blk.prefix}.5", blk.cout, blk.cout, None,
                                                      halves[i][0], xf[i][:, :cp], training, n_upd, save)
            h_dec, h_enc = halves[i]
            if plan.skip == "cat":
                if cat[i].dim() == 6:
                    cur = ops.CL2(h_dec, h_enc, xf[i][0], xf[i][1], True)
                else:
                    cur = CL(cat[i], 0, 2 * cp, xf[i][0], xf[i][1], True)
                cur_segs = ((blk.cout, 0), (blk.cout, cp))
            elif plan.skip == "none":
                cur = h_dec.with_xf(xf[i][0][:cp], xf[i][1][:cp])
                cur_segs = ((blk.cout, 0),)
            else:
                cur = CL(torch.empty((n, dd, hh, ww, cp), dtype=adt, device=dev), 0, cp)
                ops.skip_add(h_dec.with_xf(xf[i][0][:cp], xf[i][1][:cp]), h_enc.with_xf(xf[i][0][cp:], xf[i][1][cp:]), cur)
                cur_segs = ((blk.cout, 0),)
        imap_h, _ = self._maps(cur_segs, cur.cp, dev)
        wl, bl = P[plan.head + ".weight"], P[plan.head + ".bias"]
        w2 = wl.detach().reshape(wl.shape[0], wl.shape[1])
        out0, out1 = ops.head_fwd(cur, w2, bl.detach(), imap_h, plan.act, plan.head_mode)
        if save:
            ctx.update(recs=recs, x_cl=x_cl, cat=cat, xf=xf, pooled=pooled, dskip=dskip, dec_in=dec_in, ups=ups,
                       head_in=cur, imap_h=imap_h, center_out=center_out, dims=(n, d, h, w))
        return out0, out1, ctx

    def _replay(self, P, rec: _ConvRec):
        return ((P[rec.bn + ".running_mean"], P[rec.bn + ".running_var"], BN_MOMENTUM, BN_EPS,
                 P.get(rec.bn + ".num_batches_tracked")) if self._replay_stats else None)

    def _bwd_fin(self, P, rec: _ConvRec, device):
        counter = self._counter(rec.bn, "bwd", device)
        return None if counter is None else (P[rec.bn + ".weight"].detach(), rec.cout, self._replay(P, rec), counter)

    def _gy_like(self, ga: CL) -> CL:
        ent = self._gy_bufs.get(id(ga.buf))
        if ent is None:
            ent = self._gy_bufs[id(ga.buf)] = (ga.buf, torch.empty_like(ga.buf))
        return CL(ent[1], ga.c0, ga.cp)

    def _conv_bn_bwd(self, P, rec: _ConvRec, ga: CL, gin: Optional[CL], grads: Dict[str, torch.Tensor], ws: _WgradWs, part,
                     pre_reduced: Optional[int] = None, finalized=None, up_in: Optional[CL] = None):
        k = self.plan.k
        can = LAZY_BN and ga.cs == rec.y.cs and (not ga.lp or LAZY_BN_LP)
        if up_in is not None:
            lazy = can and (ops.lp_upconv_fused_wgrad_bn_supported(up_in.dims, up_in.cp) if ga.lp else
                            ops.upconv_fused_wgrad_bn_supported(up_in.dims, up_in.cp, ga.cp))
        elif rec.first is not None:
            lazy = can and not rec.bias and not ga.lp
        else:
            lazy = can and not rec.bias and rec.x is not None and ops.conv3d_wgrad_bn_supported(ga.dims, k, rec.x.cp, ga.cp, self.dtype)
        jobs = ws.jobs
        res = ops.bn_relu_bwd(rec.y, ga, rec.vec, P[rec.bn + ".weight"].detach(), rec.cout, part, self._replay(P, rec),
                              pre_reduced, self._counter(rec.bn, "bwd", ga.buf.device), finalized, lazy, jobs)
        grads[rec.bn + ".weight"], grads[rec.bn + ".bias"] = res[0], res[1]
        if up_in is not None:
            return (rec.y, rec.vec, res[2], self._gy_like(ga)) if lazy else None
        if rec.first is not None:
            if lazy:
                gy = self._gy_like(ga)
                grads[rec.conv + ".weight"] = ops.conv_first_wgrad_bn(rec.first, ga, rec.y, rec.vec, res[2], gy, rec.cout,
                                                                      ws.take(), jobs)
                ga = gy
            else:
                grads[rec.conv + ".weight"] = ops.conv_first_wgrad(rec.first, ga, rec.cout, ws.take(), jobs)
            return ops.conv_first_bwd_data(ga, P[rec.conv + ".weight"].detach(), rec.cin) if gin is not None else None
        if lazy:
            gy = self._gy_like(ga)
            grads[rec.conv + ".weight"] = ops.conv3d_wgrad_bn(rec.x, ga, rec.y, rec.vec, res[2], gy, rec.cout, rec.cin, k,
                                                             rec.imap, ws.take(), jobs)
            ga = gy
        elif rec.x is not None:
            dw, dbias = ops.conv3d_wgrad(rec.x, ga, rec.cout, rec.cin, k, rec.imap, ws.take(), rec.bias, jobs)
            grads[rec.conv + ".weight"] = dw
            if rec.bias:
                grads[rec.conv + ".bias"] = dbias
        if gin is not None:
# ... 7 lines not shown
        recs = ctx["recs"]
        n, d, h, w = ctx["dims"]
        dev = g0.device
        nlev = len(plan.enc)
        gs = 1.0
        flag = None
        dyn = self.scaler if self.dtype == torch.float16 else None
        if dyn is not None:
            dyn.prepare(dev, n * d * h * w)
            flag = dyn.found_inf
        elif self.dtype == torch.float16:
            gs = self.loss_scale if self.loss_scale else float(2 ** max(0, (n * d * h * w).bit_length() - 5))
            flag = self.overflow_flag(dev)
            flag.zero_()
        grads: Dict[str, torch.Tensor] = {}
        emitted: set = set()
        self._gy_bufs = {}

        def unscale(tensors):
            if dyn is not None:
                ops.unscale_tensors(tensors, dyn.scale, flag)
            elif gs != 1.0:
                ops.scale_tensors(tensors, 1.0 / gs, flag)

        def emit():
            new = [(nm, g) for nm, g in grads.items() if nm not in emitted and g is not None]
            emitted.update(nm for nm, _ in new)
            if sync is not None or dyn is not None or gs != 1.0:
                ws.flush()
            unscale([g for _, g in new])
            if sync is not None:
                sync.push(new)
        k = plan.k
        ws_n, part_n = 1, 1
        for r in recs.values():
            if r is None:
                continue
            if r.first is not None:
                ws_n = max(ws_n, ops.conv_first_wgrad_ws(r.y.dims, r.cin))
                part_n = max(part_n, ops.bn_bwd_partials_floats(r.y.nvox, r.y.cp))
                continue
            ws_n = max(ws_n, ops.conv3d_wgrad_ws(r.y.dims, k, r.x.cp if r.x is not None else pad8(r.cin), r.y.cp, self.dtype))
            part_n = max(part_n, ops.bn_bwd_partials_floats(r.y.nvox, r.y.cp))
        for x_in, blk in zip(ctx["dec_in"], plan.dec):
            ws_n = max(ws_n, ops.convt_wgrad_ws(x_in.dims, x_in.cp, pad8(blk.cin), self.dtype))
        for dsk in ctx["dskip"]:
            part_n = max(part_n, ops.maxpool_bwd_bn_blocks(dsk.dims, dsk.cp) * 2 * dsk.cp)
        part_n = max(part_n, ops.head_bwd_blocks(ctx["head_in"].dims) * 2 * pad8(plan.dec[-1].cout))
        ws = _WgradWs(ws_n, dev, DEFER_WGRAD_REDUCE and self.dtype == torch.float32 and ops.TIMER is None)
        part = torch.empty(part_n, dtype=torch.float32, device=dev)

        self._replay_stats = bool(ctx["training"] and ctx["chk"])

        cat, head_in = ctx["cat"], ctx["head_in"]
        gcat = [torch.empty_like(c) for c in cat]
        ghalves = [_cat_halves(g, g.shape[-1] // (1 if g.dim() == 6 else 2)) for g in gcat]
        wl, bl = P[plan.head + ".weight"], P[plan.head + ".bias"]
        w2 = wl.detach().reshape(wl.shape[0], wl.shape[1])
        gsd = None if dyn is None else dyn.scale
        def g_skip_target(level: int) -> CL:
            g_dec, g_enc = ghalves[level]
            if plan.skip != "cat":
                return g_dec
            return ops.CL2(g_dec, g_enc) if gcat[level].dim() == 6 else CL(gcat[level], 0, 2 * g_dec.cp)

        def g_skip_fanout(level: int):
            if plan.skip == "add":
                ops.skip_add(ghalves[level][0], None, ghalves[level][1])

        r_last = recs[(plan.dec[-1].prefix, 2)]
        head_rows, head_fin = None, None
        head_lo = head_in.a if isinstance(head_in, ops.CL2) else head_in
        if (POOL_BN and head_in.scale is not None and head_in.relu and head_in.scale.data_ptr() == r_last.vec[0].data_ptr()
                and head_lo.c0 == r_last.y.c0 and head_lo.buf is r_last.y.buf):
            fin = self._bwd_fin(P, r_last, dev)
            res = ops.head_bwd(head_in, w2, bl.detach(), ctx["imap_h"], plan.act, plan.head_mode, g0.contiguous(),
                               None if g1 is None else g1.contiguous(), g_skip_target(0), (r_last.vec, part), fin, gscale=gs,
                               gscale_dev=gsd)
            dwl, dbl, head_rows = res[:3]
            head_fin = res[3] if fin is not None else None
        else:
            dwl, dbl = ops.head_bwd(head_in, w2, bl.detach(), ctx["imap_h"], plan.act, plan.head_mode, g0.contiguous(),
                                    None if g1 is None else g1.contiguous(), g_skip_target(0), gscale=gs,
                                    gscale_dev=gsd)
        g_skip_fanout(0)
        grads[plan.head + ".weight"], grads[plan.head + ".bias"] = dwl.reshape(wl.shape), dbl
        emit()

        g_deep: Optional[CL] = None
        for j in range(nlev - 1, -1, -1):
            blk = plan.dec[j]
            i = nlev - 1 - j
            cp = pad8(blk.cout)
            r1, r2 = recs[(blk.prefix, 1)], recs[(blk.prefix, 2)]
            g_u2 = ghalves[i][0]
            g_u1 = CL(torch.empty_like(r1.y.buf), 0, cp)
            self._conv_bn_bwd(P, r2, g_u2, g_u1, grads, ws, part, head_rows if j == nlev - 1 else None,
                              head_fin if j == nlev - 1 else None)
            x_in = ctx["dec_in"][j]
            ct = blk.cin
            if j > 0 and plan.skip == "cat":
                segs = ((plan.dec[j - 1].cout, 0), (plan.dec[j - 1].cout, pad8(plan.dec[j - 1].cout)))
            else:
                segs = ((ct, 0),)
            imap_t, cinv_t = self._maps(segs, x_in.cp, dev)
            wt = P[f"{blk.prefix}.0.weight"]
            up = ctx["ups"][j]
            if j > 0:
                gin = g_skip_target(i + 1)
            else:
                gin = CL(torch.empty_like(x_in.buf), 0, x_in.cp)
                g_deep = gin
            if up is None:
                lz = self._conv_bn_bwd(P, r1, g_u1, None, grads, ws, part, up_in=x_in)
                gq = g_u1
                up_wgrad = ops.lp_upconv_fused_wgrad if g_u1.lp else ops.upconv_fused_wgrad
                dwt, dbt, dw3 = up_wgrad(x_in, gq, ct, blk.cout, P[f"{blk.prefix}.0.bias"], self._up_cache[blk.prefix][4], imap_t, lz)
# ... 142 lines not shown
```

### ct-unet_amd/ctunet_amd/ops.py

```python
from __future__ import annotations

import contextlib
import ctypes
import gc
import os

from dataclasses import dataclass
from typing import Optional, Sequence, Tuple

import torch

from . import _lib


def pad8(c: int) -> int:
    return (c + 7) // 8 * 8


LP_CODE = {torch.bfloat16: 1, torch.float16: 2}
ACT_DTYPES = (torch.float32, torch.bfloat16, torch.float16)


def _need_cuda(t: torch.Tensor, name: str) -> None:
    if not t.is_cuda:
# ... 217 lines not shown
            self.cp = self.buf.shape[-1] - self.c0
        assert self.buf.dim() == 5 and self.buf.is_contiguous() and self.buf.dtype in ACT_DTYPES
        assert self.cp % 8 == 0 and self.c0 % 4 == 0 and self.c0 + self.cp <= self.buf.shape[-1]
        assert self.buf.dtype == torch.float32 or (self.c0 % 8 == 0 and self.buf.shape[-1] % 8 == 0)

    @property
    def dtype(self) -> torch.dtype:
        return self.buf.dtype

    @property
    def lp(self) -> int:
        return LP_CODE.get(self.buf.dtype, 0)

    @property
    def cs(self) -> int:
        return self.buf.shape[-1]

    @property
    def dims(self) -> Tuple[int, int, int, int]:
        n, d, h, w, _ = self.buf.shape
        return n, d, h, w

    @property
    def nvox(self) -> int:
        n, d, h, w = self.dims
        return n * d * h * w

    @property
    def ptr(self):
        return _ptr(self.buf, self.c0)

    def slice(self, c0: int, cp: int) -> "CL":
        sc = None if self.scale is None else self.scale[c0:c0 + cp]
        sh = None if self.shift is None else self.shift[c0:c0 + cp]
        return CL(self.buf, self.c0 + c0, cp, sc, sh, self.relu)

    def raw(self) -> "CL":
        return CL(self.buf, self.c0, self.cp)

    def with_xf(self, scale, shift, relu=True) -> "CL":
        return CL(self.buf, self.c0, self.cp, scale, shift, relu)


@dataclass
class CL2:
    a: CL
    b: CL
    scale: Optional[torch.Tensor] = None
    shift: Optional[torch.Tensor] = None
    relu: bool = False

    def __post_init__(self):
        assert self.a.cp == self.b.cp and self.a.dims == self.b.dims and self.a.dtype == self.b.dtype
        assert self.a.cp in (8, 16), "the two-segment head kernels take at most 16 channels per segment"

    @property
    def cp(self) -> int:
        return 2 * self.a.cp

    @property
    def lp(self) -> int:
        return self.a.lp

    @property
    def dims(self) -> Tuple[int, int, int, int]:
        return self.a.dims

    def seg_args(self):
        return self.a.ptr, self.a.cs, self.b.ptr, self.b.cs


def new_cl(n, d, h, w, cs, device, zero=False, dtype=torch.float32) -> torch.Tensor:
    f = torch.zeros if zero else torch.empty
    return f((n, d, h, w, cs), dtype=dtype, device=device)


def ncdhw_to_cl(x: torch.Tensor, cp: Optional[int] = None, dtype=torch.float32) -> CL:
    _need_cuda(x, "input")
    x = x.contiguous()
    n, c, d, h, w = x.shape
    cp = cp or pad8(c)
    out = new_cl(n, d, h, w, cp, x.device, dtype=dtype)
    _dual(lp(dtype), "ncdhw_to_ndhwc", x.data_ptr(), out.data_ptr(), n, c, d, h, w, cp, cp, _stream())
    return CL(out, 0, cp)


def cl_to_ncdhw(a: CL, c: int) -> torch.Tensor:
    n, d, h, w = a.dims
    out = torch.empty((n, c, d, h, w), dtype=torch.float32, device=a.buf.device)
    _dual(a.lp, "ndhwc_to_ncdhw", a.ptr, out.data_ptr(), n, c, d, h, w, a.cs, _stream())
    return out


def conv_layout(k: int, nout_p: int, w: int, dtype=torch.float32, rin_p: int = 0) -> int:
    if lp(dtype):
        return _lib.load().ctu_lp_conv3d_layout(k, rin_p, nout_p, w)
    return _lib.load().ctu_conv3d_layout(k, nout_p, w)


def pack_conv_w(w: torch.Tensor, cinv: Optional[torch.Tensor], rin_p: int, nout_p: int, mode: int,
                layout: int = 0) -> torch.Tensor:
    _need_cuda(w, "conv weight")
    co, ci, k = w.shape[0], w.shape[1], w.shape[2]
    lib = _lib.load()
    n = lib.ctu_conv3d_packed_floats(k, rin_p, nout_p, layout)
    wp = torch.empty(n, dtype=torch.float32, device=w.device)
    _lib.check(lib.ctu_pack_conv3d_weight(w.contiguous().data_ptr(), wp.data_ptr(), co, ci, k, _ptr(cinv), rin_p,
                                          nout_p, mode, layout, _stream()), "pack_conv3d_weight")
    return wp


def packed_floats(kind: str, k: int, rin_p: int, nout_p: int, layout: int) -> int:
    lib = _lib.load()
    return lib.ctu_conv3d_packed_floats(k, rin_p, nout_p, layout) if kind == "conv" else \
        lib.ctu_convt_packed_floats(rin_p, nout_p)


def pack_batch(jobs, dtype: torch.dtype = torch.float32) -> None:
    if not jobs:
        return
    code = 0 if dtype == torch.float32 else LP_CODE[dtype]
    arr = (_lib.PackJob * len(jobs))()
# ... 349 lines not shown
        assert not x.lp or (out.dtype == x.dtype and wp.dtype == x.dtype)
        _dual(x.lp, "convt2_fwd", x.ptr, x.cs, x.cp, _ptr(x.scale), _ptr(x.shift), int(x.relu), wp.data_ptr(), _ptr(bias),
              0 if bias is None else bias.numel(), out.ptr, out.cs, out.cp, n, d, h, w, _stream())


def convt_bwd_data(gout: CL, wp: torch.Tensor, gin: CL) -> None:
    n, d, h, w = gin.dims
    with _convt_bracket("convt2_bwd_data", gout, gin.cp, gout.cp, gin.dims):
        assert not gout.lp or (gin.dtype == gout.dtype and wp.dtype == gout.dtype)
        _dual(gout.lp, "convt2_bwd_data", gout.ptr, gout.cs, gout.cp, wp.data_ptr(), gin.ptr, gin.cs, gin.cp, n, d, h, w,
              _stream())


def convt_wgrad(x: CL, g: CL, ci: int, co: int, imap, ws: torch.Tensor, jobs: Optional[WgradJobs] = None):
    n, d, h, w = x.dims
    if _deferred(jobs, x.lp):
        assert ws.numel() >= convt_wgrad_ws(x.dims, x.cp, g.cp, x.dtype)
        dw = torch.empty((ci, co, 2, 2, 2), dtype=torch.float32, device=x.buf.device)
        db = torch.empty(co, dtype=torch.float32, device=x.buf.device)
        job = _lib.WgradJob()
        _dual(0, "convt2_wgrad_slabs", x.ptr, x.cs, x.cp, _ptr(x.scale), _ptr(x.shift), int(x.relu), g.ptr, g.cs, g.cp,
              dw.data_ptr(), db.data_ptr(), ci, co, _ptr(imap), ws.data_ptr(), n, d, h, w, ctypes.byref(job), _stream())
        jobs.add(job, ws, dw, db, imap)
        return dw, db
    with _convt_bracket("convt2_wgrad", x, x.cp, g.cp, x.dims):
        assert not x.lp or g.dtype == x.dtype
        assert ws.numel() >= convt_wgrad_ws(x.dims, x.cp, g.cp, x.dtype)
        dw = torch.empty((ci, co, 2, 2, 2), dtype=torch.float32, device=x.buf.device)
        db = None if x.lp else torch.empty(co, dtype=torch.float32, device=x.buf.device)
        _dual(x.lp, "convt2_wgrad", x.ptr, x.cs, x.cp, _ptr(x.scale), _ptr(x.shift), int(x.relu), g.ptr, g.cs, g.cp,
              dw.data_ptr(), *(() if x.lp else (db.data_ptr(),)), ci, co, _ptr(imap), ws.data_ptr(), n, d, h, w, _stream())
        if x.lp:
            db = channel_sum(g, co)
    return dw, db


def convt_wgrad_ws(dims, cin_p, cout_p, dtype=torch.float32) -> int:
    n, d, h, w = dims
    return _query(lp(dtype), "convt2_wgrad_ws_floats", n, d, h, w, cin_p, cout_p)


def head_fwd(x, w: torch.Tensor, b: torch.Tensor, imap, act: int, head_mode: int):
    n, d, h, w_ = x.dims
    co, ci = w.shape[0], w.shape[1]
    v = d * h * w_
    dev = w.device
    if head_mode == 0:
        out0 = torch.empty((n, co, d, h, w_), dtype=torch.float32, device=dev)
        out1 = None
    else:
        out0 = torch.empty((n, 2, d, h, w_), dtype=torch.float32, device=dev)
        out1 = torch.empty((n, 2, d, h, w_), dtype=torch.float32, device=dev)
    seg2 = isinstance(x, CL2)
    src = (*x.seg_args(), x.a.cp) if seg2 else (x.ptr, x.cs, x.cp)
    _dual(x.lp, "head_fwd_seg2" if seg2 else "head_fwd", *src, _ptr(x.scale), _ptr(x.shift), int(x.relu), w.data_ptr(),
          b.data_ptr(), _ptr(imap), ci, co, act, head_mode, out0.data_ptr(), _ptr(out1), n, v, _stream())
    return out0, out1


def head_bwd(x, w: torch.Tensor, b: torch.Tensor, imap, act: int, head_mode: int, g0: torch.Tensor,
             g1: Optional[torch.Tensor], gin, bn=None, fin=None, gscale: float = 1.0,
             gscale_dev: Optional[torch.Tensor] = None):
    assert gscale == 1.0 or x.lp, "gscale is the 16-bit path's loss scale"
    assert gscale_dev is None or (x.lp and gscale_dev.is_cuda and gscale_dev.dtype == torch.float32), \
        "gscale_dev is the 16-bit path's device loss scale"
    n, d, h, w_ = x.dims
    co, ci = w.shape[0], w.shape[1]
    v = d * h * w_
    dev = w.device
    seg2 = isinstance(x, CL2)
    assert seg2 == isinstance(gin, CL2), "head_bwd: input and input gradient are both one buffer or both two segments"
    lib = _lib.load()
    ws = torch.empty(lib.ctu_head_bwd_ws_floats(n, v, x.cp, co), dtype=torch.float32, device=dev)
    dw = torch.empty_like(w)
    db = torch.empty_like(b)
    bn_args, tail, done = (None, None, 0, None), None, None
    if bn is not None:
        vec, partials = bn
        bn_cp = vec.shape[1]
        rows = lib.ctu_head_bwd_num_blocks(n, v)
        assert x.scale is not None and x.relu and vec[0].data_ptr() == x.scale.data_ptr() and partials.numel() >= rows * 2 * bn_cp
        bn_args = (vec[2].data_ptr(), vec[3].data_ptr(), bn_cp, partials.data_ptr())
        if fin is not None:
            gamma, c, replay = fin[:3]
            tail, done = _bn_bwd_outputs(c, bn_cp, n * v, gamma, vec, replay, None, dev)
    entry, scale = "head_bwd_bn", ((float(gscale),) if x.lp else ())
    if gscale_dev is not None:
        entry, scale = "head_bwd_bn_dscale", (gscale_dev.data_ptr(),)
    if seg2:
        entry, src, dst = entry + "_seg2", (*x.seg_args(), x.a.cp), gin.seg_args()
    else:
        src, dst = (x.ptr, x.cs, x.cp), (gin.ptr, gin.cs)
    _dual(x.lp, entry, *src, _ptr(x.scale), _ptr(x.shift), int(x.relu), w.data_ptr(), b.data_ptr(), _ptr(imap),
          ci, co, act, head_mode, g0.data_ptr(), _ptr(g1), *dst, dw.data_ptr(), db.data_ptr(), ws.data_ptr(), n, v,
          *bn_args, _tail_arg(tail), *scale, _stream())
    if bn is None:
        return dw, db
    return (dw, db, rows) if fin is None else (dw, db, rows, done)


def head_bwd_blocks(dims) -> int:
    n, d, h, w_ = dims
    return _lib.load().ctu_head_bwd_num_blocks(n, d * h * w_)


def loss_fwd(pred: torch.Tensor, target: torch.Tensor, ce_lambda: float, dice_lambda: float, dice_softmax: bool):
    _need_cuda(pred, "prediction")
    _need_cuda(target, "target")
    assert pred.shape == target.shape and pred.shape[1] == 2, "loss kernel handles 2-channel maps"
    pred, target = pred.contiguous(), target.contiguous()
    n = pred.shape[0]
    v = pred[0, 0].numel()
    lib = _lib.load()
    ws = torch.empty(lib.ctu_loss_ws_floats(n, v), dtype=torch.float32, device=pred.device)
    terms = torch.empty(2, dtype=torch.float32, device=pred.device)
    _lib.check(lib.ctu_loss_fwd(pred.data_ptr(), target.data_ptr(), n, v, ce_lambda, dice_lambda, int(dice_softmax),
                                terms.data_ptr(), ws.data_ptr(), _stream()), "loss_fwd")
    return terms, ws


def loss_bwd(pred, target, ce_lambda, dice_lambda, dice_softmax, ws, g_ce: Optional[torch.Tensor],
             g_dice: Optional[torch.Tensor], out: Optional[torch.Tensor] = None, accumulate: bool = False) -> torch.Tensor:
    pred, target = pred.contiguous(), target.contiguous()
    for g_ in (g_ce, g_dice):
# ... 34 lines not shown
def seg_loss_fwd(pred: torch.Tensor, target: torch.Tensor, lambdas: Sequence[float], dice_softmax: bool,
                 class_weight: Sequence[float] = (1.0, 1.0), focal_gamma: float = 0.0,
                 tversky_ab: Sequence[float] = (0.5, 0.5), boundary: Optional[torch.Tensor] = None):
    pred, target, boundary, n, v, cfg = _seg_loss_args(pred, target, lambdas, dice_softmax, class_weight, focal_gamma,
                                                      tversky_ab, boundary)
    lib = _lib.load()
    ws = torch.empty(lib.ctu_seg_loss_ws_floats(n, v), dtype=torch.float32, device=pred.device)
    terms = torch.empty(4, dtype=torch.float32, device=pred.device)
    _lib.check(lib.ctu_seg_loss_fwd(pred.data_ptr(), target.data_ptr(), _ptr(boundary), n, v, ctypes.byref(cfg),
                                    terms.data_ptr(), ws.data_ptr(), _stream()), "seg_loss_fwd")
    return terms, ws


def seg_loss_bwd(pred, target, lambdas, dice_softmax, ws, upstream: Sequence[Optional[torch.Tensor]] = (None,) * 4,
                 class_weight: Sequence[float] = (1.0, 1.0), focal_gamma: float = 0.0,
                 tversky_ab: Sequence[float] = (0.5, 0.5), boundary: Optional[torch.Tensor] = None,
                 out: Optional[torch.Tensor] = None, accumulate: bool = False) -> torch.Tensor:
    pred, target, boundary, n, v, cfg = _seg_loss_args(pred, target, lambdas, dice_softmax, class_weight, focal_gamma,
                                                      tversky_ab, boundary)
    assert len(upstream) == 4
    for g_ in upstream:
        assert g_ is None or (g_.is_cuda and g_.dtype == torch.float32 and g_.numel() == 1)
    g = out if out is not None else torch.empty_like(pred)
    lib = _lib.load()
    _lib.check(lib.ctu_seg_loss_bwd(pred.data_ptr(), target.data_ptr(), _ptr(boundary), n, v, ctypes.byref(cfg),
                                    ws.data_ptr(), *(_ptr(g_) for g_ in upstream), g.data_ptr(), int(accumulate),
                                    _stream()), "seg_loss_bwd")
    return g



def skip_add(a: CL, b: Optional[CL], out: CL) -> None:
    assert out.dims == a.dims and out.cp == a.cp and (b is None or (b.dims == a.dims and b.cp == a.cp))
    assert out.dtype == a.dtype and (b is None or b.dtype == a.dtype)
    _dual(a.lp, "skip_add", a.ptr, a.cs, _ptr(a.scale), _ptr(a.shift), int(a.relu), 0 if b is None else b.ptr,
          0 if b is None else b.cs, _ptr(b.scale) if b is not None else 0, _ptr(b.shift) if b is not None else 0,
          int(b.relu) if b is not None else 0, out.ptr, out.cs, out.cp, a.nvox, _stream())


def channel_sum(x: CL, c: int) -> torch.Tensor:
    lib = _lib.load()
    nb = lib.ctu_channel_sum_num_blocks(x.nvox)
    part = torch.empty(nb * x.cp, dtype=torch.float32, device=x.buf.device)
    out = torch.empty(c, dtype=torch.float32, device=x.buf.device)
    _dual(x.lp, "channel_sum", x.ptr, x.cs, x.cp, x.nvox, part.data_ptr(), out.data_ptr(), c, _stream())
    return out


def upconv_fused_supported(dims, k: int, cin_p: int, nout_p: int) -> bool:
    n, d, h, w = dims
    return bool(_lib.load().ctu_upconv_fused_supported(k, d, h, w, cin_p, nout_p))


def upconv_fused_pack(wt: torch.Tensor, bt: torch.Tensor, w3: torch.Tensor, cinv, cin_p: int, nout_p: int,
                      into=None):
    return _upconv_pack(wt, bt, w3, cinv, cin_p, nout_p, into, False)


def upconv_fused_pack_all(wt: torch.Tensor, bt: torch.Tensor, w3: torch.Tensor, cinv, cin_p: int, nout_p: int,
                          into=None):
    return _upconv_pack(wt, bt, w3, cinv, cin_p, nout_p, into, True)


def _upconv_pack(wt, bt, w3, cinv, cin_p, nout_p, into, with_wpd: bool):
    lib = _lib.load()
    c, co = wt.shape[0], w3.shape[0]
    assert wt.shape == (c, c, 2, 2, 2) and w3.shape == (co, c, 3, 3, 3) and bt.shape == (c,)
    if into is not None:
        bufs = tuple(into)
        assert len(bufs) == 3 + with_wpd
    else:
        new = lambda n: torch.empty(n, dtype=torch.float32, device=wt.device)
        bufs = (new(lib.ctu_upconv_fused_packed_floats(cin_p, nout_p)), new((27, nout_p)),
                new(lib.ctu_upconv_fused_pack_ws_floats(c, nout_p)))
        if with_wpd:
            bufs += (new(lib.ctu_upconv_fused_bwd_packed_floats(cin_p, nout_p)),)
    wp, beff, ws = bufs[:3]
    _lib.check(lib.ctu_upconv_fused_pack_all(wt.detach().contiguous().data_ptr(), bt.detach().contiguous().data_ptr(),
                                             w3.detach().contiguous().data_ptr(), c, co, _ptr(cinv), cin_p, nout_p, wp.data_ptr(),
                                             beff.data_ptr(), ws.data_ptr(), bufs[3].data_ptr() if with_wpd else None, _stream()),
               "upconv_fused_pack")
    return bufs


def upconv_fused_num_blocks(dims, nout_p: int) -> int:
    n, d, h, w = dims
    return _lib.load().ctu_upconv_fused_num_blocks(n, d, h, w, nout_p)


def upconv_fused_fwd(x: CL, wp: torch.Tensor, beff: torch.Tensor, out: CL, stats: Optional[torch.Tensor],
                     algo_ch: Optional[Tuple[int, int]] = None, tail=None) -> None:
    n, d, h, w = x.dims
    assert out.dims == (n, 2 * d, 2 * h, 2 * w)
    ci, co = algo_ch if algo_ch is not None else (x.cp, out.cp)
    vox = n * d * h * w
    with _timed(lambda: (f"upconv_fused_fwd_kernel<{out.cp}>", vox * (16.0 * ci * ci + 8 * 54.0 * ci * co),
                         4.0 * vox * (ci + 8 * co), (w, x.cp, out.cp))):
        _lib.check(_lib.load().ctu_upconv_fused_fwd(x.ptr, x.cs, x.cp, _ptr(x.scale), _ptr(x.shift), int(x.relu),
                                                    wp.data_ptr(), beff.data_ptr(), out.ptr, out.cs, out.cp, _ptr(stats),
                                                    n, d, h, w, _tail_arg(tail), _stream()), "upconv_fused_fwd")


def upconv_fused_wgrad_bn_supported(dims, cin_p: int, nout_p: int, dtype=torch.float32) -> bool:
    n, d, h, w = dims
    return dtype == torch.float32 and bool(_lib.load().ctu_upconv_fused_wgrad_bn_supported(n, d, h, w, cin_p, nout_p))


def upconv_fused_wgrad(x: CL, g: CL, c: int, co: int, bt: torch.Tensor, pack_ws: torch.Tensor, imap, lazy=None):
    n, d, h, w = x.dims
    assert g.dims == (n, 2 * d, 2 * h, 2 * w) and not x.lp
    return _upconv_wgrad(x, g, c, co, bt, pack_ws, imap, lazy,
                         lambda: (f"upconv_fused_wgrad_kernel<{g.cp}> (+slab reduce)", 4.0 * (n * d * h * w) * (c + 8 * co)))


def _upconv_wgrad(x: CL, g: CL, c: int, co: int, bt, pack_ws, imap, lazy, tag_bytes):
    n, d, h, w = x.dims
    dev = x.buf.device
    gcp = () if x.lp else (g.cp,)
    dweff = torch.empty((8, 8, x.cp, g.cp), dtype=torch.float32, device=dev)
    ws = torch.empty(_query(x.lp, "upconv_fused_wgrad_ws_floats", n, d, h, w, x.cp, *gcp), dtype=torch.float32, device=dev)
    act = (x.ptr, x.cs, x.cp, _ptr(x.scale), _ptr(x.shift), int(x.relu), g.ptr, g.cs, *gcp)
    detail = (w, x.cp, g.cp)

    def record():
        tag, nbytes = tag_bytes()
        return tag, (n * d * h * w) * (16.0 * c * c + 8 * 54.0 * c * co), nbytes, detail
    with _timed(record):
        if lazy is not None:
            y, vec, coef, gy = lazy
            assert y.dims == g.dims and gy.dims == g.dims and y.cs == g.cs == gy.cs and y.cp == g.cp == gy.cp
            assert gy.buf.data_ptr() != g.buf.data_ptr()
            _dual(x.lp, "upconv_fused_wgrad_bn", *act, y.ptr, vec[0].data_ptr(), vec[1].data_ptr(), coef.data_ptr(), gy.ptr,
                  dweff.data_ptr(), ws.data_ptr(), n, d, h, w, _stream())
            g = gy
        else:
            _dual(x.lp, "upconv_fused_wgrad", *act, dweff.data_ptr(), ws.data_ptr(), n, d, h, w, _stream())
    dwt = torch.empty((c, c, 2, 2, 2), dtype=torch.float32, device=dev)
    dbt = torch.empty(c, dtype=torch.float32, device=dev)
    dw3 = torch.empty((co, c, 3, 3, 3), dtype=torch.float32, device=dev)
    ws2 = torch.empty(_lib.load().ctu_upconv_fused_project_ws_floats(g.cp, g.nvox), dtype=torch.float32, device=dev)
    _dual(x.lp, "upconv_fused_project", dweff.data_ptr(), g.ptr, g.cs, g.cp, n, d, h, w, bt.detach().data_ptr(),
          pack_ws.data_ptr(), _ptr(imap), c, co, x.cp, dwt.data_ptr(), dbt.data_ptr(), dw3.data_ptr(), ws2.data_ptr(), _stream())
    return dwt, dbt, dw3


def lp_upconv_fused_supported(dims, k: int, cin_p: int, nout_p: int) -> bool:
    n, d, h, w = dims
    return bool(_lib.load().ctu_lp_upconv_fused_supported(k, d, h, w, cin_p, nout_p))


def lp_upconv_fused_pack(wp32: torch.Tensor, cin_p: int, dtype: torch.dtype, into: Optional[torch.Tensor] = None) -> torch.Tensor:
    lib = _lib.load()
    n = lib.ctu_lp_upconv_fused_packed_elems(cin_p)
    wp16 = into if into is not None else torch.empty(n, dtype=dtype, device=wp32.device)
    assert wp16.numel() == n and wp16.dtype == dtype
    _lib.check(lib.ctu_lp_upconv_fused_pack(LP_CODE[dtype], wp32.data_ptr(), cin_p, wp16.data_ptr(), _stream()), "lp_upconv_fused_pack")
    return wp16


def lp_upconv_fused_num_blocks(dims) -> int:
    n, d, h, w = dims
    return _lib.load().ctu_lp_upconv_fused_num_blocks(n, d, h, w)


def lp_upconv_fused_fwd(x: CL, wp16: torch.Tensor, beff: torch.Tensor, out: CL, stats: Optional[torch.Tensor],
                        algo_ch: Optional[Tuple[int, int]] = None) -> None:
    n, d, h, w = x.dims
    assert out.dims == (n, 2 * d, 2 * h, 2 * w) and x.lp and out.dtype == x.dtype and wp16.dtype == x.dtype and out.cp == 8
    ci, co = algo_ch if algo_ch is not None else (x.cp, out.cp)
    vox = n * d * h * w
    with _timed(lambda: (f"lp_upconv_fwd_kernel<{_lp_name(x.lp)}>", vox * (16.0 * ci * ci + 8 * 54.0 * ci * co),
                         2.0 * vox * (x.cp + 8 * out.cp), (w, x.cp, out.cp))):
        _lib.check(_lib.load().ctu_lp_upconv_fused_fwd(x.lp, x.ptr, x.cs, x.cp, _ptr(x.scale), _ptr(x.shift), int(x.relu),
                                                       wp16.data_ptr(), beff.data_ptr(), out.ptr, out.cs, _ptr(stats),
                                                       n, d, h, w, _stream()), "lp_upconv_fused_fwd")


def lp_upconv_fused_wgrad_bn_supported(dims, cin_p: int) -> bool:
    n, d, h, w = dims
    return bool(_lib.load().ctu_lp_upconv_fused_wgrad_bn_supported(n, d, h, w, cin_p))


def lp_upconv_fused_wgrad(x: CL, g: CL, c: int, co: int, bt: torch.Tensor, pack_ws: torch.Tensor, imap, lazy=None):
    n, d, h, w = x.dims
    assert g.dims == (n, 2 * d, 2 * h, 2 * w) and x.lp and g.dtype == x.dtype and g.cp == 8 and g.cs == 8
    return _upconv_wgrad(x, g, c, co, bt, pack_ws, imap, lazy,
                         lambda: (f"lp_upconv_wgrad_kernel<{_lp_name(x.lp)}> (+slab reduce)", 2.0 * (n * d * h * w) * (x.cp + 8 * g.cp)))


def lp_upconv_fused_bwd_data(g: CL, wp16: torch.Tensor, gin: CL, algo_ch: Optional[Tuple[int, int]] = None) -> None:
    n, d, h, w = gin.dims
    assert g.dims == (n, 2 * d, 2 * h, 2 * w) and g.lp and gin.dtype == g.dtype and wp16.dtype == g.dtype and g.cp == 8
    ci, co = algo_ch if algo_ch is not None else (gin.cp, g.cp)
    vox = n * d * h * w
    with _timed(lambda: (f"lp_upconv_bwd_data_kernel<{_lp_name(g.lp)}>", vox * (16.0 * ci * ci + 8 * 54.0 * ci * co),
                         2.0 * vox * (gin.cp + 8 * g.cp), (w, gin.cp, g.cp))):
        _lib.check(_lib.load().ctu_lp_upconv_fused_bwd_data(g.lp, g.ptr, g.cs, wp16.data_ptr(), gin.ptr, gin.cs, gin.cp,
                                                            n, d, h, w, _stream()), "lp_upconv_fused_bwd_data")


def upconv_fused_pack_bwd(wp: torch.Tensor, cin_p: int, nout_p: int, into: Optional[torch.Tensor] = None) -> torch.Tensor:
    lib = _lib.load()
    wpd = into if into is not None else torch.empty(lib.ctu_upconv_fused_bwd_packed_floats(cin_p, nout_p),
                                                     dtype=torch.float32, device=wp.device)
    _lib.check(lib.ctu_upconv_fused_pack_bwd(wp.data_ptr(), cin_p, nout_p, wpd.data_ptr(), _stream()), "upconv_fused_pack_bwd")
    return wpd


def upconv_fused_bwd_data(g: CL, wpd: torch.Tensor, gin: CL, algo_ch: Optional[Tuple[int, int]] = None) -> None:
    n, d, h, w = gin.dims
    assert g.dims == (n, 2 * d, 2 * h, 2 * w)
    ci, co = algo_ch if algo_ch is not None else (gin.cp, g.cp)
    vox = n * d * h * w
    with _timed(lambda: (f"upconv_fused_bwd_data_kernel<{g.cp}>", vox * (16.0 * ci * ci + 8 * 54.0 * ci * co),
                         4.0 * vox * (ci + 8 * co), (w, gin.cp, g.cp))):
        _lib.check(_lib.load().ctu_upconv_fused_bwd_data(g.ptr, g.cs, g.cp, wpd.data_ptr(), gin.ptr, gin.cs, gin.cp,
                                                         n, d, h, w, _stream()), "upconv_fused_bwd_data")


def _ncv(t: torch.Tensor):
    if t.dtype != torch.float32 or not t.is_cuda or not t.is_contiguous() or t.dim() not in (4, 5):
        raise RuntimeError("ctunet_amd: expected a contiguous float32 CUDA map [N,C,D,H,W] or [C,D,H,W]")
    n = t.shape[0] if t.dim() == 5 else 1
    c = t.shape[1] if t.dim() == 5 else t.shape[0]
    return n, c, t.numel() // (n * c)


def hard_segm(prob: torch.Tensor) -> torch.Tensor:
    n, c, v = _ncv(prob)
    out = torch.empty(prob.shape[:1] + prob.shape[2:] if prob.dim() == 5 else prob.shape[1:], dtype=torch.float32,
                      device=prob.device)
    _lib.check(_lib.load().ctu_hard_segm(prob.data_ptr(), n, c, v, out.data_ptr(), _stream()), "hard_segm")
    return out


def one_hot(label: torch.Tensor, num_classes: int) -> torch.Tensor:
    if label.dtype != torch.float32 or not label.is_cuda or not label.is_contiguous() or label.dim() != 4:
        raise RuntimeError("ctunet_amd: expected a contiguous float32 CUDA label volume [N,D,H,W]")
    n = label.shape[0]
    out = torch.empty((n, num_classes) + tuple(label.shape[1:]), dtype=torch.float32, device=label.device)
    _lib.check(_lib.load().ctu_one_hot(label.data_ptr(), n, num_classes, label.numel() // n, out.data_ptr(), _stream()),
               "one_hot")
    return out


def hard_dice_counts(pred: torch.Tensor, target: torch.Tensor) -> torch.Tensor:
    n, c, v = _ncv(pred)
    if target.shape != pred.shape or _ncv(target) != (n, c, v):
        raise RuntimeError("ctunet_amd: prediction and one-hot target must have the same shape")
    lib = _lib.load()
    ws = torch.empty(lib.ctu_hard_dice_ws_doubles(n), dtype=torch.float64, device=pred.device)
    counts = torch.empty((n, c, 3), dtype=torch.float64, device=pred.device)
    _lib.check(lib.ctu_hard_dice_counts(pred.data_ptr(), target.data_ptr(), n, c, v, counts.data_ptr(), ws.data_ptr(),
                                        _stream()), "hard_dice_counts")
    return counts


def hausdorff(pred: torch.Tensor, target: torch.Tensor) -> torch.Tensor:
    n, c, v = _ncv(pred)
    if pred.dim() != 5 or target.shape != pred.shape or _ncv(target) != (n, c, v):
        raise RuntimeError("ctunet_amd: hausdorff expects a [N,C,D,H,W] prediction and a one-hot target of the same shape")
    d, h, w = pred.shape[2:]
    lib = _lib.load()
    ws = torch.empty(lib.ctu_hausdorff_ws_bytes(n, c, d, h, w), dtype=torch.uint8, device=pred.device)
    out = torch.empty((n, c - 1), dtype=torch.float32, device=pred.device)
    _lib.check(lib.ctu_hausdorff(pred.data_ptr(), target.data_ptr(), n, c, d, h, w, out.data_ptr(), ws.data_ptr(), _stream()),
               "hausdorff")
    return out


# ... 273 lines not shown
```

### include/ctunet_hip.h

```cpp
#ifndef CTUNET_HIP_H
#define CTUNET_HIP_H

#include <stddef.h>
#include <stdint.h>

#ifdef __cplusplus
extern "C" {
#endif

#define CTU_OK 0
#define CTU_EINVAL (-1)
#define CTU_ELAUNCH (-2)

#define CTU_F32 0
#define CTU_BF16 1
#define CTU_F16 2

typedef struct ctu_bn_tail {
    const float* gamma; const float* beta;
    float* running_mean; float* running_var;
    float* scale; float* shift; float* mean; float* invstd;
    long long* num_batches_tracked;
    unsigned int* counter;
    double count;
// ... 191 lines not shown
int ctu_loss_fwd(const float* pred, const float* target, int N, int64_t V, float ce_lambda,
                 float dice_lambda, int dice_softmax, float* terms, float* ws, void* stream);
int ctu_loss_bwd(const float* pred, const float* target, int N, int64_t V, float ce_lambda,
                 float dice_lambda, int dice_softmax, const float* ws, const float* gscale_ce,
                 const float* gscale_dice, float* gpred, int accumulate, void* stream);

typedef struct ctu_seg_loss_cfg {
    float ce_lambda, dice_lambda, tversky_lambda, boundary_lambda;
    float w0, w1;
    float focal_gamma;
    float tversky_alpha, tversky_beta;
    int dice_softmax;
} ctu_seg_loss_cfg;
size_t ctu_seg_loss_ws_floats(int N, int64_t V);
int ctu_seg_loss_fwd(const float* pred, const float* target, const float* phi, int N, int64_t V,
                     const ctu_seg_loss_cfg* cfg, float* terms, float* ws, void* stream);
int ctu_seg_loss_bwd(const float* pred, const float* target, const float* phi, int N, int64_t V,
                     const ctu_seg_loss_cfg* cfg, const float* ws, const float* g_ce, const float* g_dice,
                     const float* g_tversky, const float* g_boundary, float* gpred, int accumulate, void* stream);

int ctu_skip_add(const float* a, int a_cs, const float* a_scale, const float* a_shift, int a_relu,
                 const float* b, int b_cs, const float* b_scale, const float* b_shift, int b_relu,
                 float* out, int out_cs, int cp, int64_t nvox, void* stream);
int ctu_upconv_fused_supported(int k, int D, int H, int W, int cin_p, int nout_p);
size_t ctu_upconv_fused_packed_floats(int cin_p, int nout_p);
int ctu_upconv_fused_num_blocks(int N, int D, int H, int W, int nout_p);
size_t ctu_upconv_fused_pack_ws_floats(int C, int nout_p);
int ctu_upconv_fused_pack(const float* wt, const float* bt, const float* w3, int C, int Co, const int32_t* cinv,
                          int cin_p, int nout_p, float* wp, float* beff, float* ws, void* stream);
int ctu_upconv_fused_pack_all(const float* wt, const float* bt, const float* w3, int C, int Co, const int32_t* cinv,
                              int cin_p, int nout_p, float* wp, float* beff, float* ws, float* wpd, void* stream);
int ctu_upconv_fused_fwd(const float* in, int in_cs, int cin_p, const float* in_scale, const float* in_shift,
                         int in_relu, const float* wp, const float* beff, float* out, int out_cs, int nout_p,
                         float* stats, int N, int D, int H, int W, const ctu_bn_tail* tail, void* stream);

size_t ctu_upconv_fused_wgrad_ws_floats(int N, int D, int H, int W, int cin_p, int nout_p);
int ctu_upconv_fused_wgrad(const float* in, int in_cs, int cin_p, const float* in_scale, const float* in_shift,
                           int in_relu, const float* gout, int g_cs, int nout_p, float* dweff, float* ws,
                           int N, int D, int H, int W, void* stream);
int ctu_upconv_fused_wgrad_bn_supported(int N, int D, int H, int W, int cin_p, int nout_p);
int ctu_upconv_fused_wgrad_bn(const float* in, int in_cs, int cin_p, const float* in_scale, const float* in_shift,
                              int in_relu, const float* ga, int g_cs, int nout_p, const float* y,
                              const float* bn_scale, const float* bn_shift, const float* coef, float* gy_out,
                              float* dweff, float* ws, int N, int D, int H, int W, void* stream);
size_t ctu_upconv_fused_project_ws_floats(int nout_p, int64_t fine_nvox);
int ctu_upconv_fused_project(const float* dweff, const float* gout, int g_cs, int nout_p, int N, int D, int H, int W,
                             const float* bt, const float* pack_ws, const int32_t* imap, int C, int Co, int cin_p,
                             float* dwt, float* dbt, float* dw3, float* ws, void* stream);

size_t ctu_upconv_fused_bwd_packed_floats(int cin_p, int nout_p);
int ctu_upconv_fused_pack_bwd(const float* wp, int cin_p, int nout_p, float* wpd, void* stream);
int ctu_upconv_fused_bwd_data(const float* gout, int g_cs, int nout_p, const float* wpd, float* gin, int gin_cs,
                              int cin_p, int N, int D, int H, int W, void* stream);

int ctu_hard_segm(const float* prob, int N, int C, int64_t nvox_per_item, float* seg, void* stream);
int ctu_one_hot(const float* label, int N, int C, int64_t nvox_per_item, float* out, void* stream);
size_t ctu_hard_dice_ws_doubles(int N);
int ctu_hard_dice_counts(const float* pred, const float* target, int N, int C, int64_t nvox_per_item,
                         double* counts, double* ws, void* stream);

size_t ctu_hausdorff_ws_bytes(int N, int C, int D, int H, int W);
int ctu_hausdorff(const float* pred, const float* target, int N, int C, int D, int H, int W, float* out, void* ws,
                  void* stream);

#define CTU_U8 3
#define CTU_I64 4
size_t ctu_surface_ws_bytes(int N, int Cs, int D, int H, int W);
int ctu_surface_metrics(const void* pred, int pred_dtype, int pred_onehot, const void* target, int target_dtype,
                        int target_onehot, int N, int C, int cls0, int Cs, int D, int H, int W, const float* spacing,
                        const double* tau, double percentile, float* out, void* ws, void* stream);

#define CTU_CC_LARGEST 0
#define CTU_CC_MIN_SIZE 1
size_t ctu_components_ws_bytes(int N, int D, int H, int W);
int ctu_label_components(const void* in, int dtype, int N, int D, int H, int W, int connectivity, const int64_t* applied,
                         int n_applied, int32_t* labels, int32_t* num, void* ws, void* stream);
int ctu_filter_components(const void* in, int dtype, int N, int D, int H, int W, int connectivity,
                          const int64_t* applied, int n_applied, int mode, int param, void* out, void* ws, void* stream);

#define CTU_MORPH_ERODE 0
#define CTU_MORPH_DILATE 1
#define CTU_MORPH_OPEN 2
#define CTU_MORPH_CLOSE 3
#define CTU_MORPH_WS_MORPH 0
#define CTU_MORPH_WS_FILL 1
#define CTU_MORPH_WS_IMPLANT 2
size_t ctu_morphology_ws_bytes(int N, int D, int H, int W, int kind);
int ctu_binary_morphology(const void* in, int dtype, int N, int D, int H, int W, int mode, uint32_t structure,
                          int iterations, int border, int has_label, int64_t label, uint8_t* out, void* ws, void* stream);
int ctu_fill_holes(const void* in, int dtype, int N, int D, int H, int W, int connectivity, int has_label, int64_t label,
                   uint8_t* out, void* ws, void* stream);
int ctu_implant_mask(const void* full, int full_dtype, const void* defective, int defective_dtype, int N, int D, int H,
                     int W, uint32_t structure, int opening_iterations, int fill_holes, int connectivity,
                     int num_components, uint8_t* out, void* ws, void* stream);

#define CTU_DIST_EDT 0
#define CTU_DIST_SQUARED 1
#define CTU_DIST_SIGNED 2
#define CTU_DIST_BALL 3
size_t ctu_distance_ws_bytes(int N, int D, int H, int W, int out_kind, int want_indices);
int ctu_distance_transform(const void* in, int dtype, int N, int D, int H, int W, int has_label, int64_t label, int invert,
                           int border_background, const float* spacing, int out_kind, void* out, int32_t* indices,
                           float ball_r2, void* ws, void* stream);

size_t ctu_thickness_ws_bytes(int N, int D, int H, int W, int is_float);
int ctu_local_thickness(const void* d2, int is_float, int N, int D, int H, int W, const float* spacing, void* out, void* ws,
// ... 339 lines not shown
```

Measured before the change: 712.8 million voxels/s.

## Let fused up-convolution kernels read and write two channel segments directly

Adds two-segment (concatenated skip + upsampled) variants of the fused up-convolution forward, weight-gradient and backward-data kernels. Each kernel now picks its base pointer per channel tile, so the concatenated tensor never has to be materialised. This is meant to remove a concat copy and its gradient split in the decoder, at the cost of extra template instantiations and a per-tile branch. It only helps if the Python model path builds CL2 inputs for these layers.

```diff
diff --git a/ct-unet_amd/csrc/conv3d.hip b/ct-unet_amd/csrc/conv3d.hip
--- a/ct-unet_amd/csrc/conv3d.hip
+++ b/ct-unet_amd/csrc/conv3d.hip
@@ -1054,6 +1054,10 @@
     const float* lz_coef;
     int lz_cp;
 };
+struct WgP2 : WgP {
+    const float* in1;
+    int seg_c;
+};
 
 template <int KS, int KDS, int TD, int TH, int TW>
 __global__ __launch_bounds__(256, CTU_WG_OCC) void conv3d_wgrad_kernel(WgP p) {
@@ -1216,9 +1220,11 @@
 }
 
 
-template <int SM, int SN, int UP = 0, bool LZ = false>
-__global__ __launch_bounds__(256, CTU_K3S_OCC) void conv3d_wgrad_k3s_kernel(WgP p, int tiles_per_block) {
+template <int SM, int SN, int UP = 0, bool LZ = false, bool S2 = false>
+__global__ __launch_bounds__(256, CTU_K3S_OCC) void conv3d_wgrad_k3s_kernel(typename std::conditional<S2, WgP2, WgP>::type p,
+                                                                            int tiles_per_block) {
     static_assert(!UP || (SM == 1 && SN == 1), "the fused up-convolution uses the full 16 x 16 channel tile");
+    static_assert(!S2 || UP, "two input segments: the fused up-convolution only");
     constexpr int TD = 4, TH = 4, TW = (SM == 2 && SN == 2) ? 16 : 8, HD = 6, HH = 6, HW = TW + 2, HV = HD * HH * HW;
     constexpr int KPR = TW / 4, NKS = TH * KPR;
     constexpr int CM = 16 / SM, CN = 16 / SN;
@@ -1318,7 +1324,11 @@
     auto prep = [&](Box b) -> bool {
         const int d0 = b.tz * TD, h0 = b.ty * TH, w0 = b.tx * TW;
         const long long org = (((long long)b.n * p.D + d0) * p.H + h0) * p.W + w0;
-        pf_abase = reinterpret_cast<const char*>(p.in + (org - ((long long)p.H * p.W + p.W + 1)) * p.in_cs);
+        const float* src = p.in;
+        if constexpr (S2) {
+            if (ci0 >= p.seg_c) src = p.in1 - p.seg_c;
+        }
+        pf_abase = reinterpret_cast<const char*>(src + (org - ((long long)p.H * p.W + p.W + 1)) * p.in_cs);
         if (UP) {
             const long long gorg = (((long long)b.n * 2 * p.D + 2 * d0 + pz) * gH + 2 * h0 + py) * gW + 2 * w0 + px;
             pf_gbase = reinterpret_cast<const char*>(p.g + gorg * p.g_cs);
@@ -2275,38 +2285,71 @@
     return na > nb ? na : nb;
 }
 
-static int upconv_fused_wgrad_impl(const float* in, int in_cs, int cin_p, const float* in_scale, const float* in_shift,
-                                   int in_relu, const float* gout, int g_cs, int nout_p, float* dweff, float* ws,
-                                   int N, int D, int H, int W, const LazyBn* lz, void* stream);
+static int upconv_fused_wgrad_impl(const float* in, const float* in1, int seg_c, int in_cs, int cin_p, const float* in_scale,
+                                   const float* in_shift, int in_relu, const float* gout, int g_cs, int nout_p, float* dweff,
+                                   float* ws, int N, int D, int H, int W, const LazyBn* lz, void* stream);
 
 extern "C" int ctu_upconv_fused_wgrad(const float* in, int in_cs, int cin_p, const float* in_scale, const float* in_shift,
                                       int in_relu, const float* gout, int g_cs, int nout_p, float* dweff, float* ws,
                                       int N, int D, int H, int W, void* stream) {
-    return upconv_fused_wgrad_impl(in, in_cs, cin_p, in_scale, in_shift, in_relu, gout, g_cs, nout_p, dweff, ws, N, D, H, W,
-                                   nullptr, stream);
+    return upconv_fused_wgrad_impl(in, nullptr, 0, in_cs, cin_p, in_scale, in_shift, in_relu, gout, g_cs, nout_p, dweff, ws,
+                                   N, D, H, W, nullptr, stream);
 }
 
 extern "C" int ctu_upconv_fused_wgrad_bn_supported(int N, int D, int H, int W, int cin_p, int nout_p) {
     return (N > 0 && D % 4 == 0 && H % 4 == 0 && W % 8 == 0 && cin_p % 16 == 0 && nout_p % 8 == 0) ? 1 : 0;
 }
+
+#define CTU_UPWG_BN_CHECK(name)                                                                                              \
+    CTU_REQUIRE(y && bn_scale && bn_shift && coef && gy_out, name ": null pointer");                                         \
+    CTU_REQUIRE(ctu_upconv_fused_wgrad_bn_supported(N, D, H, W, cin_p, nout_p), name ": geometry not supported");            \
+    CTU_REQUIRE(((uintptr_t)y & 15) == 0 && ((uintptr_t)gy_out & 15) == 0 && gy_out != ga,                                   \
+                name ": y / gy_out alignment, gy_out must not alias ga")
 
 extern "C" int ctu_upconv_fused_wgrad_bn(const float* in, int in_cs, int cin_p, const float* in_scale, const float* in_shift,
                                          int in_relu, const float* ga, int g_cs, int nout_p, const float* y,
                                          const float* bn_scale, const float* bn_shift, const float* coef, float* gy_out,
                                          float* dweff, float* ws, int N, int D, int H, int W, void* stream) {
-    CTU_REQUIRE(y && bn_scale && bn_shift && coef && gy_out, "upconv_fused_wgrad_bn: null pointer");
-    CTU_REQUIRE(ctu_upconv_fused_wgrad_bn_supported(N, D, H, W, cin_p, nout_p), "upconv_fused_wgrad_bn: geometry not supported");
-    CTU_REQUIRE(((uintptr_t)y & 15) == 0 && ((uintptr_t)gy_out & 15) == 0 && gy_out != ga, "upconv_fused_wgrad_bn: y / gy_out alignment, gy_out must not alias ga");
+    CTU_UPWG_BN_CHECK("upconv_fused_wgrad_bn");
     const LazyBn lz = {y, bn_scale, bn_shift, coef, gy_out, nout_p};
-    return upconv_fused_wgrad_impl(in, in_cs, cin_p, in_scale, in_shift, in_relu, ga, g_cs, nout_p, dweff, ws, N, D, H, W, &lz, stream);
-}
-
-static int upconv_fused_wgrad_impl(const float* in, int in_cs, int cin_p, const float* in_scale, const float* in_shift,
-                                   int in_relu, const float* gout, int g_cs, int nout_p, float* dweff, float* ws,
-                                   int N, int D, int H, int W, const LazyBn* lz, void* stream) {
+    return upconv_fused_wgrad_impl(in, nullptr, 0, in_cs, cin_p, in_scale, in_shift, in_relu, ga, g_cs, nout_p, dweff, ws,
+                                   N, D, H, W, &lz, stream);
+}
+
+#define CTU_UPWG_SEG2_CHECK(name)                                                                                            \
+    CTU_REQUIRE(in0 && in1, name ": null segment");                                                                          \
+    CTU_REQUIRE(seg_c > 0 && seg_c % 16 == 0 && 2 * seg_c == cin_p,                                                          \
+                name ": seg_c=%d must be a multiple of 16 and half of cin_p=%d", seg_c, cin_p);                              \
+    CTU_REQUIRE(((uintptr_t)in1 & 15) == 0, name ": 16-byte alignment")
+
+extern "C" int ctu_upconv_fused_wgrad_seg2(const float* in0, const float* in1, int seg_c, int cs, int cin_p, const float* in_scale,
+                                           const float* in_shift, int in_relu, const float* gout, int g_cs, int nout_p,
+                                           float* dweff, float* ws, int N, int D, int H, int W, void* stream) {
+    CTU_UPWG_SEG2_CHECK("upconv_fused_wgrad_seg2");
+    return upconv_fused_wgrad_impl(in0, in1, seg_c, cs, cin_p, in_scale, in_shift, in_relu, gout, g_cs, nout_p, dweff, ws,
+                                   N, D, H, W, nullptr, stream);
+}
+
+extern "C" int ctu_upconv_fused_wgrad_bn_seg2(const float* in0, const float* in1, int seg_c, int cs, int cin_p,
+                                              const float* in_scale, const float* in_shift, int in_relu, const float* ga, int g_cs,
+                                              int nout_p, const float* y, const float* bn_scale, const float* bn_shift,
+                                              const float* coef, float* gy_out, float* dweff, float* ws, int N, int D, int H,
+                                              int W, void* stream) {
+    CTU_UPWG_SEG2_CHECK("upconv_fused_wgrad_bn_seg2");
+    CTU_UPWG_BN_CHECK("upconv_fused_wgrad_bn_seg2");
+    const LazyBn lz = {y, bn_scale, bn_shift, coef, gy_out, nout_p};
+    return upconv_fused_wgrad_impl(in0, in1, seg_c, cs, cin_p, in_scale, in_shift, in_relu, ga, g_cs, nout_p, dweff, ws,
+                                   N, D, H, W, &lz, stream);
+}
+#undef CTU_UPWG_SEG2_CHECK
+#undef CTU_UPWG_BN_CHECK
+
+static int upconv_fused_wgrad_impl(const float* in, const float* in1, int seg_c, int in_cs, int cin_p, const float* in_scale,
+                                   const float* in_shift, int in_relu, const float* gout, int g_cs, int nout_p, float* dweff,
+                                   float* ws, int N, int D, int H, int W, const LazyBn* lz, void* stream) {
     CTU_REQUIRE(in && gout && dweff && ws, "upconv_fused_wgrad: null pointer");
     CTU_REQUIRE(cin_p % 8 == 0 && nout_p % 8 == 0 && cin_p > 0 && nout_p > 0 && nout_p <= 64, "upconv_fused_wgrad: padded channels");
-    CTU_REQUIRE(in_cs >= cin_p && in_cs % 4 == 0 && g_cs >= nout_p && g_cs % 4 == 0, "upconv_fused_wgrad: bad stride");
+    CTU_REQUIRE(in_cs >= (seg_c ? seg_c : cin_p) && in_cs % 4 == 0 && g_cs >= nout_p && g_cs % 4 == 0, "upconv_fused_wgrad: bad stride");
     CTU_REQUIRE(((uintptr_t)in & 15) == 0 && ((uintptr_t)gout & 15) == 0, "upconv_fused_wgrad: 16-byte alignment");
     CTU_REQUIRE((in_scale == nullptr) == (in_shift == nullptr), "upconv_fused_wgrad: scale/shift must come together");
     CTU_REQUIRE((int64_t)(2 * H * W + 2 * W + 2) * in_cs * 4 < (int64_t)1 << 31 && (int64_t)(8 * 2 * H + 8) * 2 * W * g_cs * 4 < (int64_t)1 << 31,
@@ -2314,7 +2357,8 @@
     hipStream_t st = (hipStream_t)stream;
     const bool pw = nout_p == 8 && g_cs == 8;
     const UpWgPlan g = upwg_plan(N, D, H, W, cin_p, nout_p, pw);
-    WgP p;
+    WgP2 p;
+    p.in1 = in1; p.seg_c = seg_c;
     p.in = in; p.in_scale = in_scale; p.in_shift = in_shift; p.g = gout; p.ws = ws;
     p.in_cs = in_cs; p.cin_p = cin_p; p.in_relu = in_relu; p.g_cs = g_cs; p.cout_p = nout_p;
     p.N = N; p.D = D; p.H = H; p.W = W;
@@ -2322,17 +2366,24 @@
     p.ntiles = g.ntiles; p.n_ci_t = g.n_ci_g; p.n_co_t = g.n_co_g;
     p.lz_y = nullptr; p.lz_out = nullptr; p.lz_scale = nullptr; p.lz_shift = nullptr; p.lz_coef = nullptr; p.lz_cp = 0;
     if (lz) { p.lz_y = lz->y; p.lz_out = lz->out; p.lz_scale = lz->scale; p.lz_shift = lz->shift; p.lz_coef = lz->coef; p.lz_cp = lz->cp; }
+    const dim3 grid(g.grid.gx, g.pairs);
+#define CTU_UPWG_LAUNCH(UP)                                                                                              \
+    do {                                                                                                                 \
+        if (seg_c && lz) conv3d_wgrad_k3s_kernel<1, 1, UP, true, true><<<grid, 256, 0, st>>>(p, g.grid.tpb);              \
+        else if (seg_c) conv3d_wgrad_k3s_kernel<1, 1, UP, false, true><<<grid, 256, 0, st>>>(p, g.grid.tpb);              \
+        else if (lz) conv3d_wgrad_k3s_kernel<1, 1, UP, true><<<grid, 256, 0, st>>>(p, g.grid.tpb);                        \
+        else conv3d_wgrad_k3s_kernel<1, 1, UP><<<grid, 256, 0, st>>>(p, g.grid.tpb);                                      \
+    } while (0)
     if (pw) {
         p.cout_p = 16;
-        if (lz) conv3d_wgrad_k3s_kernel<1, 1, 2, true><<<dim3(g.grid.gx, g.pairs), 256, 0, st>>>(p, g.grid.tpb);
-        else conv3d_wgrad_k3s_kernel<1, 1, 2><<<dim3(g.grid.gx, g.pairs), 256, 0, st>>>(p, g.grid.tpb);
+        CTU_UPWG_LAUNCH(2);
         CTU_CHECK_LAUNCH("upconv_fused_wgrad(pw)");
         upconv_wgrad_reduce_pw_kernel<<<dim3(12 * 256 / 64, g.pairs), 64 * RPARTS, 0, st>>>(ws, dweff, cin_p, g.n_ci_g, g.grid.gx);
         CTU_CHECK_LAUNCH("upconv_fused_wgrad_reduce(pw)");
         return CTU_OK;
     }
-    if (lz) conv3d_wgrad_k3s_kernel<1, 1, 1, true><<<dim3(g.grid.gx, g.pairs), 256, 0, st>>>(p, g.grid.tpb);
-    else conv3d_wgrad_k3s_kernel<1, 1, 1><<<dim3(g.grid.gx, g.pairs), 256, 0, st>>>(p, g.grid.tpb);
+    CTU_UPWG_LAUNCH(1);
+#undef CTU_UPWG_LAUNCH
     CTU_CHECK_LAUNCH("upconv_fused_wgrad");
     upconv_wgrad_reduce_kernel<<<dim3(8 * 256 / 64, g.pairs), 64 * RPARTS, 0, st>>>(ws, dweff, cin_p, nout_p, g.n_ci_g, g.n_co_g, g.grid.gx);
     CTU_CHECK_LAUNCH("upconv_fused_wgrad_reduce");
diff --git a/ct-unet_amd/csrc/upconv_fused.hip b/ct-unet_amd/csrc/upconv_fused.hip
--- a/ct-unet_amd/csrc/upconv_fused.hip
+++ b/ct-unet_amd/csrc/upconv_fused.hip
@@ -21,8 +21,15 @@
     ctu_bn_tail tail;
 };
 
-template <int PB, int NTP, bool PW = false>
-__global__ __launch_bounds__(256, 2) void upconv_fused_fwd_kernel(UpP p, int ntiles, int tiles_per_block) {
+template <class P>
+struct UpSeg2 : P {
+    float* seg1;
+    int seg_c;
+};
+
+template <int PB, int NTP, bool PW = false, bool S2 = false>
+__global__ __launch_bounds__(256, 2) void upconv_fused_fwd_kernel(typename std::conditional<S2, UpSeg2<UpP>, UpP>::type p, int ntiles,
+                                                                   int tiles_per_block) {
     static_assert(PW ? (PB == 4 && NTP == 1) : ((PB * NTP == 8 || (PB == 4 && NTP == 1)) && (PB == 8 || PB == 4 || PB == 2)), "tile-parities per block");
     constexpr int NTW = PW ? 3 : 2, TAPS = 4 * NTW;
     constexpr int MT = 4, TD = 4, TH = 4, TW = 16;
@@ -109,7 +116,11 @@
             sh = *reinterpret_cast<const float4*>(p.in_shift + cc * 8 + half * 4);
         }
         const long long org = (((long long)b.n * p.D + d0) * p.H + h0) * p.W + w0 - ((long long)p.H * p.W + p.W + 1);
-        const char* base = reinterpret_cast<const char*>(p.in + org * p.in_cs + cc * 8);
+        const float* src = p.in;
+        if constexpr (S2) {
+            if (cc * 8 >= p.seg_c) src = p.seg1 - p.seg_c;
+        }
+        const char* base = reinterpret_cast<const char*>(src + org * p.in_cs + cc * 8);
         a_interior = d0 >= 1 && h0 >= 1 && w0 >= 1 && d0 + TD < p.D && h0 + TH < p.H && w0 + TW < p.W;
         if (a_interior) {
 #pragma unroll
@@ -318,8 +329,9 @@
     int tiles_d, tiles_h, tiles_w, n16;
 };
 
-template <int NT>
-__global__ __launch_bounds__(256, 2) void upconv_fused_bwd_data_kernel(UpDP p, int ntiles, int tiles_per_block) {
+template <int NT, bool S2 = false>
+__global__ __launch_bounds__(256, 2) void upconv_fused_bwd_data_kernel(typename std::conditional<S2, UpSeg2<UpDP>, UpDP>::type p,
+                                                                        int ntiles, int tiles_per_block) {
     constexpr int MT = 4, TD = 4, TH = 4, TW = 16;
     constexpr int HD = TD + 2, HH = TH + 2, HW = TW + 2, HV = HD * HH * HW;
     constexpr int NTHR = 256;
@@ -525,17 +537,22 @@
         if (c == nchunk - 1) {
             const int d0 = box.tz * TD, h0 = box.ty * TH, w0 = box.tx * TW;
             const int gw = w0 + m;
-            float* obase = p.out + ((((size_t)box.n * p.D + d0 + wave) * p.H + h0) * p.W + gw) * p.out_cs;
+            const size_t ovox = (((size_t)box.n * p.D + d0 + wave) * p.H + h0) * p.W + gw;
+            float* obase = p.out + ovox * p.out_cs;
             const int orow = p.W * p.out_cs;
 #pragma unroll
             for (int nt = 0; nt < NT; ++nt) {
                 const int co = (by * NT + nt) * 16 + kq * 4;
+                float* otile = obase;
+                if constexpr (S2) {
+                    if ((by * NT + nt) * 16 >= p.seg_c) otile = p.seg1 - p.seg_c + ovox * p.out_cs;
+                }
 #pragma unroll
                 for (int mt = 0; mt < MT; ++mt) {
                     if (co < p.cin_p && d0 + wave < p.D && h0 + mt < p.H && gw < p.W) {
                         float4 o;
                         o.x = acc[mt][nt][0]; o.y = acc[mt][nt][1]; o.z = acc[mt][nt][2]; o.w = acc[mt][nt][3];
-                        *reinterpret_cast<float4*>(obase + mt * orow + co) = o;
+                        *reinterpret_cast<float4*>(otile + mt * orow + co) = o;
                     }
                     acc[mt][nt] = f32x4{0.f, 0.f, 0.f, 0.f};
                 }
@@ -948,19 +965,26 @@
     return ctu_upconv_fused_pack_all(wt, bt, w3, C, Co, cinv, cin_p, nout_p, wp, beff, ws, nullptr, stream);
 }
 
-extern "C" int ctu_upconv_fused_fwd(const float* in, int in_cs, int cin_p, const float* in_scale, const float* in_shift,
-                                    int in_relu, const float* wp, const float* beff, float* out, int out_cs, int nout_p,
-                                    float* stats, int N, int D, int H, int W, const ctu_bn_tail* tail, void* stream) {
+static bool up_seg2_ok(int cin_p, int seg_c, int mult) { return seg_c > 0 && seg_c % mult == 0 && 2 * seg_c == cin_p; }
+
+extern "C" int ctu_upconv_fused_seg2_supported(int k, int D, int H, int W, int cin_p, int nout_p, int seg_c) {
+    return ctu_upconv_fused_supported(k, D, H, W, cin_p, nout_p) && up_seg2_ok(cin_p, seg_c, 16);
+}
+
+static int upconv_fused_fwd_impl(const float* in, const float* in1, int seg_c, int in_cs, int cin_p, const float* in_scale,
+                                 const float* in_shift, int in_relu, const float* wp, const float* beff, float* out, int out_cs,
+                                 int nout_p, float* stats, int N, int D, int H, int W, const ctu_bn_tail* tail, void* stream) {
     CTU_REQUIRE(in && wp && beff && out, "upconv_fused_fwd: null pointer");
     CTU_REQUIRE(ctu_upconv_fused_supported(3, D, H, W, cin_p, nout_p), "upconv_fused_fwd: unsupported geometry (W=%d cin_p=%d nout_p=%d)",
                 W, cin_p, nout_p);
-    CTU_REQUIRE(in_cs >= cin_p && in_cs % 4 == 0 && out_cs >= nout_p && out_cs % 4 == 0, "upconv_fused_fwd: bad stride");
+    CTU_REQUIRE(in_cs >= (seg_c ? seg_c : cin_p) && in_cs % 4 == 0 && out_cs >= nout_p && out_cs % 4 == 0, "upconv_fused_fwd: bad stride");
     CTU_REQUIRE((in_scale == nullptr) == (in_shift == nullptr), "upconv_fused_fwd: scale/shift must come together");
     CTU_REQUIRE(((uintptr_t)in & 15) == 0 && ((uintptr_t)out & 15) == 0 && ((uintptr_t)wp & 15) == 0 && ((uintptr_t)beff & 15) == 0,
                 "upconv_fused_fwd: 16-byte alignment");
     CTU_REQUIRE((int64_t)N * D * H * W * 8 < (int64_t)1 << 31 && (int64_t)(2 * H * W + 2 * W + 2) * in_cs * 4 < (int64_t)1 << 31,
                 "upconv_fused_fwd: volume too large for 32-bit offsets");
-    UpP p;
+    UpSeg2<UpP> p;
+    p.seg1 = const_cast<float*>(in1); p.seg_c = seg_c;
     p.in = in; p.in_scale = in_scale; p.in_shift = in_shift; p.wp = wp; p.beff = beff; p.out = out; p.stats = stats;
     CTU_REQUIRE(!tail || (stats && tail->counter && tail->gamma && tail->beta && tail->scale && tail->shift && tail->mean &&
                           tail->invstd && tail->C > 0 && tail->C <= nout_p && tail->count > 0),
@@ -972,16 +996,40 @@
     p.tiles_d = r.tiles_d; p.tiles_h = r.tiles_h; p.tiles_w = r.tiles_w;
     const int ny = r.ny, gx = r.grid.gx, tpb = r.grid.tpb, ntiles = r.ntiles;
     hipStream_t st = (hipStream_t)stream;
+#define CTU_UP_FWD(NY, ...)                                                                                            \
+    do {                                                                                                               \
+        if (seg_c) upconv_fused_fwd_kernel<__VA_ARGS__, true><<<dim3(gx, NY), 256, 0, st>>>(p, ntiles, tpb);            \
+        else upconv_fused_fwd_kernel<__VA_ARGS__, false><<<dim3(gx, NY), 256, 0, st>>>(p, ntiles, tpb);                 \
+    } while (0)
     if (nout_p == 16 && ny == 2) {
-        upconv_fused_fwd_kernel<4, 1><<<dim3(gx, 2), 256, 0, st>>>(p, ntiles, tpb);
+        CTU_UP_FWD(2, 4, 1, false);
     } else if (nout_p == 8) {
         p.wp = wp + up_std_packed(cin_p, nout_p);
-        upconv_fused_fwd_kernel<4, 1, true><<<dim3(gx, 1), 256, 0, st>>>(p, ntiles, tpb);
-    } else if (ny == 1) upconv_fused_fwd_kernel<8, 1><<<dim3(gx, 1), 256, 0, st>>>(p, ntiles, tpb);
-    else if (ny == 2) upconv_fused_fwd_kernel<4, 2><<<dim3(gx, 2), 256, 0, st>>>(p, ntiles, tpb);
-    else upconv_fused_fwd_kernel<2, 4><<<dim3(gx, 4), 256, 0, st>>>(p, ntiles, tpb);
+        CTU_UP_FWD(1, 4, 1, true);
+    } else if (ny == 1) CTU_UP_FWD(1, 8, 1, false);
+    else if (ny == 2) CTU_UP_FWD(2, 4, 2, false);
+    else CTU_UP_FWD(4, 2, 4, false);
+#undef CTU_UP_FWD
     CTU_CHECK_LAUNCH("upconv_fused_fwd");
     return CTU_OK;
+}
+
+extern "C" int ctu_upconv_fused_fwd(const float* in, int in_cs, int cin_p, const float* in_scale, const float* in_shift,
+                                    int in_relu, const float* wp, const float* beff, float* out, int out_cs, int nout_p,
+                                    float* stats, int N, int D, int H, int W, const ctu_bn_tail* tail, void* stream) {
+    return upconv_fused_fwd_impl(in, nullptr, 0, in_cs, cin_p, in_scale, in_shift, in_relu, wp, beff, out, out_cs, nout_p, stats,
+                                 N, D, H, W, tail, stream);
+}
+
+extern "C" int ctu_upconv_fused_fwd_seg2(const float* in0, const float* in1, int seg_c, int cs, int cin_p, const float* in_scale,
+                                         const float* in_shift, int in_relu, const float* wp, const float* beff, float* out,
+                                         int out_cs, int nout_p, float* stats, int N, int D, int H, int W, const ctu_bn_tail* tail,
+                                         void* stream) {
+    CTU_REQUIRE(in0 && in1, "upconv_fused_fwd_seg2: null segment");
+    CTU_REQUIRE(up_seg2_ok(cin_p, seg_c, 8), "upconv_fused_fwd_seg2: seg_c=%d must be a multiple of 8 and half of cin_p=%d", seg_c, cin_p);
+    CTU_REQUIRE(((uintptr_t)in1 & 15) == 0, "upconv_fused_fwd_seg2: 16-byte alignment");
+    return upconv_fused_fwd_impl(in0, in1, seg_c, cs, cin_p, in_scale, in_shift, in_relu, wp, beff, out, out_cs, nout_p, stats,
+                                 N, D, H, W, tail, stream);
 }
 
 extern "C" int ctu_channel_sum_num_blocks(int64_t nvox);
@@ -1043,14 +1091,15 @@
     return upconv_pack_gather(wp, cin_p, nout_p, nullptr, wpd, (hipStream_t)stream);
 }
 
-extern "C" int ctu_upconv_fused_bwd_data(const float* gout, int g_cs, int nout_p, const float* wpd, float* gin, int gin_cs,
-                                         int cin_p, int N, int D, int H, int W, void* stream) {
+static int upconv_fused_bwd_data_impl(const float* gout, int g_cs, int nout_p, const float* wpd, float* gin, float* gin1, int seg_c,
+                                      int gin_cs, int cin_p, int N, int D, int H, int W, void* stream) {
     CTU_REQUIRE(gout && wpd && gin, "upconv_fused_bwd_data: null pointer");
     CTU_REQUIRE(ctu_upconv_fused_supported(3, D, H, W, cin_p, nout_p), "upconv_fused_bwd_data: unsupported geometry");
-    CTU_REQUIRE(g_cs >= nout_p && g_cs % 4 == 0 && gin_cs >= cin_p && gin_cs % 4 == 0, "upconv_fused_bwd_data: bad stride");
+    CTU_REQUIRE(g_cs >= nout_p && g_cs % 4 == 0 && gin_cs >= (seg_c ? seg_c : cin_p) && gin_cs % 4 == 0, "upconv_fused_bwd_data: bad stride");
     CTU_REQUIRE(((uintptr_t)gout & 15) == 0 && ((uintptr_t)gin & 15) == 0 && ((uintptr_t)wpd & 15) == 0, "upconv_fused_bwd_data: alignment");
     CTU_REQUIRE((int64_t)(12 * 2 * H + 12) * 2 * W * g_cs * 4 + 64 < (int64_t)1 << 31, "upconv_fused_bwd_data: volume too large for 32-bit offsets");
-    UpDP p;
+    UpSeg2<UpDP> p;
+    p.seg1 = gin1; p.seg_c = seg_c;
     p.g = gout; p.wp = wpd; p.out = gin; p.g_cs = g_cs; p.nout_p = nout_p; p.out_cs = gin_cs; p.cin_p = cin_p;
     p.N = N; p.D = D; p.H = H; p.W = W;
     p.n16 = ceil_div(cin_p, 16);
@@ -1058,9 +1107,26 @@
     p.tiles_d = r.tiles_d; p.tiles_h = r.tiles_h; p.tiles_w = r.tiles_w;
     const int NT = r.nt, ny = r.ny, gx = r.grid.gx, tpb = r.grid.tpb, ntiles = r.ntiles;
     hipStream_t st = (hipStream_t)stream;
-    if (NT == 4) upconv_fused_bwd_data_kernel<4><<<dim3(gx, ny), 256, 0, st>>>(p, ntiles, tpb);
+    if (seg_c) {
+        if (NT == 4) upconv_fused_bwd_data_kernel<4, true><<<dim3(gx, ny), 256, 0, st>>>(p, ntiles, tpb);
+        else if (NT == 2) upconv_fused_bwd_data_kernel<2, true><<<dim3(gx, ny), 256, 0, st>>>(p, ntiles, tpb);
+        else upconv_fused_bwd_data_kernel<1, true><<<dim3(gx, ny), 256, 0, st>>>(p, ntiles, tpb);
+    } else if (NT == 4) upconv_fused_bwd_data_kernel<4><<<dim3(gx, ny), 256, 0, st>>>(p, ntiles, tpb);
     else if (NT == 2) upconv_fused_bwd_data_kernel<2><<<dim3(gx, ny), 256, 0, st>>>(p, ntiles, tpb);
     else upconv_fused_bwd_data_kernel<1><<<dim3(gx, ny), 256, 0, st>>>(p, ntiles, tpb);
     CTU_CHECK_LAUNCH("upconv_fused_bwd_data");
     return CTU_OK;
 }
+
+extern "C" int ctu_upconv_fused_bwd_data(const float* gout, int g_cs, int nout_p, const float* wpd, float* gin, int gin_cs,
+                                         int cin_p, int N, int D, int H, int W, void* stream) {
+    return upconv_fused_bwd_data_impl(gout, g_cs, nout_p, wpd, gin, nullptr, 0, gin_cs, cin_p, N, D, H, W, stream);
+}
+
+extern "C" int ctu_upconv_fused_bwd_data_seg2(const float* gout, int g_cs, int nout_p, const float* wpd, float* gin0, float* gin1,
+                                              int seg_c, int cs, int cin_p, int N, int D, int H, int W, void* stream) {
+    CTU_REQUIRE(gin0 && gin1, "upconv_fused_bwd_data_seg2: null segment");
+    CTU_REQUIRE(up_seg2_ok(cin_p, seg_c, 16), "upconv_fused_bwd_data_seg2: seg_c=%d must be a multiple of 16 and half of cin_p=%d", seg_c, cin_p);
+    CTU_REQUIRE(((uintptr_t)gin1 & 15) == 0, "upconv_fused_bwd_data_seg2: alignment");
+    return upconv_fused_bwd_data_impl(gout, g_cs, nout_p, wpd, gin0, gin1, seg_c, cs, cin_p, N, D, H, W, stream);
+}
diff --git a/ct-unet_amd/ctunet_amd/_lib.py b/ct-unet_amd/ctunet_amd/_lib.py
--- a/ct-unet_amd/ctunet_amd/_lib.py
+++ b/ct-unet_amd/ctunet_amd/_lib.py
@@ -130,6 +130,11 @@
     "ctu_upconv_fused_bwd_packed_floats": (Z, [I, I]),
     "ctu_upconv_fused_pack_bwd": (I, [P, I, I, P, P]),
     "ctu_upconv_fused_bwd_data": (I, [P, I, I, P, P, I, I, I, I, I, I, P]),
+    "ctu_upconv_fused_seg2_supported": (I, [I, I, I, I, I, I, I]),
+    "ctu_upconv_fused_fwd_seg2": (I, [P, P, I, I, I, P, P, I, P, P, P, I, I, P, I, I, I, I, P, P]),
+    "ctu_upconv_fused_wgrad_seg2": (I, [P, P, I, I, I, P, P, I, P, I, I, P, P, I, I, I, I, P]),
+    "ctu_upconv_fused_wgrad_bn_seg2": (I, [P, P, I, I, I, P, P, I, P, I, I, P, P, P, P, P, P, P, I, I, I, I, P]),
+    "ctu_upconv_fused_bwd_data_seg2": (I, [P, I, I, P, P, P, I, I, I, I, I, I, I, P]),
     "ctu_hard_segm": (I, [P, I, I, L, P, P]),
     "ctu_one_hot": (I, [P, I, I, L, P, P]),
     "ctu_hard_dice_ws_doubles": (Z, [I]),
diff --git a/ct-unet_amd/ctunet_amd/engine.py b/ct-unet_amd/ctunet_amd/engine.py
--- a/ct-unet_amd/ctunet_amd/engine.py
+++ b/ct-unet_amd/ctunet_amd/engine.py
@@ -2,6 +2,7 @@
 
 import os
 from dataclasses import dataclass
+from types import SimpleNamespace
 from typing import Dict, List, Optional, Tuple
 
 import torch
@@ -20,12 +21,16 @@
 BN_TAIL = os.environ.get("CTUNET_BN_TAIL", "0") != "0"
 DEFER_WGRAD_REDUCE = os.environ.get("CTUNET_DEFER_WGRAD_REDUCE", "1") != "0"
 SPLIT_CAT0 = os.environ.get("CTUNET_SPLIT_CAT0", "1") != "0"
-
-
-def _cat_halves(buf: torch.Tensor, cp: int):
+SPLIT_CAT1 = os.environ.get("CTUNET_SPLIT_CAT1", "1") != "0"
+
+
+def _cat_halves(buf: torch.Tensor, cp: int, split: bool):
+    if not split:
+        return CL(buf, 0, cp), CL(buf, cp, cp)
     if buf.dim() == 6:
         return CL(buf[0], 0, cp), CL(buf[1], 0, cp)
-    return CL(buf, 0, cp), CL(buf, cp, cp)
+    n = buf.shape[0] // 2
+    return CL(buf[:n], 0, cp), CL(buf[n:], 0, cp)
 
 
 @dataclass
@@ -221,12 +226,22 @@
         rec = _ConvRec(x, out.raw(), vec4, stats, nblk, conv, bn, cin, cout, imap, bias is not None) if save else None
         return y, rec
 
-    def _fuse_up(self, x: CL, nout_p: int) -> bool:
+    def _fuse_up(self, x, nout_p: int) -> bool:
         if not (self.plan.k == 3 and not self.plan.conv_bias and nout_p <= FUSE_UP_MAX_CO and FUSE_UP):
             return False
         if self.dtype == torch.float32:
             return ops.upconv_fused_supported(x.dims, 3, x.cp, nout_p)
         return LP_FUSE_UP and ops.lp_upconv_fused_supported(x.dims, 3, x.cp, nout_p)
+
+    def _split_cat(self, level: int, dims, cp: int) -> bool:
+        if level == 0:
+            return SPLIT_CAT0 and cp <= 16
+        plan = self.plan
+        if not (SPLIT_CAT1 and level == 1 and plan.skip == "cat" and self.dtype == torch.float32 and cp * 4 < 128):
+            return False
+        nout_p = pad8(plan.dec[len(plan.enc) - level].cout)
+        whole = SimpleNamespace(dims=dims, cp=2 * cp)
+        return self._fuse_up(whole, nout_p) and ops.upconv_fused_seg2_supported(dims, 3, 2 * cp, nout_p, cp)
 
     def _upconv_bn(self, P, x: CL, prefix: str, ct: int, cout: int, cinv, out: CL, vec4: torch.Tensor, training: bool,
                    n_upd: int, save: bool) -> Tuple[CL, Optional[_ConvRec]]:
@@ -289,6 +304,7 @@
         cur = None if first_direct else ops.ncdhw_to_cl(x, dtype=adt)
         x_cl = cur
         cat: List[torch.Tensor] = []
+        cat_split: List[bool] = []
         halves = []
         xf: List[torch.Tensor] = []
         pooled: List[CL] = []
@@ -300,9 +316,11 @@
         xf_off = 0
         for i, blk in enumerate(plan.enc):
             cp = pad8(blk.cout)
-            split = SPLIT_CAT0 and i == 0 and cp <= 16
-            cat.append(torch.empty((2, n, dd, hh, ww, cp) if split else (n, dd, hh, ww, 2 * cp), dtype=adt, device=dev))
-            halves.append(_cat_halves(cat[i], cp))
+            split = self._split_cat(i, (n, dd, hh, ww), cp)
+            shape = (n, dd, hh, ww, 2 * cp) if not split else ((2, n, dd, hh, ww, cp) if i == 0 else (2 * n, dd, hh, ww, cp))
+            cat.append(torch.empty(shape, dtype=adt, device=dev))
+            cat_split.append(split)
+            halves.append(_cat_halves(cat[i], cp, split))
             xf.append(xf_all[xf_off:xf_off + 8 * cp].view(4, 2 * cp))
             xf_off += 8 * cp
             t1 = CL(torch.empty((n, dd, hh, ww, cp), dtype=adt, device=dev), 0, cp)
@@ -361,6 +379,7 @@
                 a1, recs[(blk.prefix, 1)] = self._upconv_bn(P, cur, blk.prefix, ct, blk.cout, cinv_t, t1, v1, training,
                                                             n_upd, save)
             else:
+                assert isinstance(cur, CL), "a split concat level feeds a fused up-convolution only"
                 up = CL(torch.empty((n, dd, hh, ww, ctp), dtype=adt, device=dev), 0, ctp)
                 wpt = self._packed(f"{blk.prefix}.0", wt, "convt", cinv_t, cur.cp, ctp, 0)
                 ops.convt_fwd(cur, wpt, P[f"{blk.prefix}.0.bias"].detach(), up)
@@ -371,7 +390,7 @@
                                                       halves[i][0], xf[i][:, :cp], training, n_upd, save)
             h_dec, h_enc = halves[i]
             if plan.skip == "cat":
-                if cat[i].dim() == 6:
+                if cat_split[i]:
                     cur = ops.CL2(h_dec, h_enc, xf[i][0], xf[i][1], True)
                 else:
                     cur = CL(cat[i], 0, 2 * cp, xf[i][0], xf[i][1], True)
@@ -388,8 +407,8 @@
         w2 = wl.detach().reshape(wl.shape[0], wl.shape[1])
         out0, out1 = ops.head_fwd(cur, w2, bl.detach(), imap_h, plan.act, plan.head_mode)
         if save:
-            ctx.update(recs=recs, x_cl=x_cl, cat=cat, xf=xf, pooled=pooled, dskip=dskip, dec_in=dec_in, ups=ups,
-                       head_in=cur, imap_h=imap_h, center_out=center_out, dims=(n, d, h, w))
+            ctx.update(recs=recs, x_cl=x_cl, cat=cat, cat_split=cat_split, xf=xf, pooled=pooled, dskip=dskip, dec_in=dec_in,
+                       ups=ups, head_in=cur, imap_h=imap_h, center_out=center_out, dims=(n, d, h, w))
         return out0, out1, ctx
 
     def _replay(self, P, rec: _ConvRec):
@@ -503,9 +522,9 @@
 
         self._replay_stats = bool(ctx["training"] and ctx["chk"])
 
-        cat, head_in = ctx["cat"], ctx["head_in"]
+        cat, cat_split, head_in = ctx["cat"], ctx["cat_split"], ctx["head_in"]
         gcat = [torch.empty_like(c) for c in cat]
-        ghalves = [_cat_halves(g, g.shape[-1] // (1 if g.dim() == 6 else 2)) for g in gcat]
+        ghalves = [_cat_halves(g, g.shape[-1] // (1 if sp else 2), sp) for g, sp in zip(gcat, cat_split)]
         wl, bl = P[plan.head + ".weight"], P[plan.head + ".bias"]
         w2 = wl.detach().reshape(wl.shape[0], wl.shape[1])
         gsd = None if dyn is None else dyn.scale
@@ -513,7 +532,7 @@
             g_dec, g_enc = ghalves[level]
             if plan.skip != "cat":
                 return g_dec
-            return ops.CL2(g_dec, g_enc) if gcat[level].dim() == 6 else CL(gcat[level], 0, 2 * g_dec.cp)
+            return ops.CL2(g_dec, g_enc) if cat_split[level] else CL(gcat[level], 0, 2 * g_dec.cp)
 
         def g_skip_fanout(level: int):
             if plan.skip == "add":
diff --git a/ct-unet_amd/ctunet_amd/ops.py b/ct-unet_amd/ctunet_amd/ops.py
--- a/ct-unet_amd/ctunet_amd/ops.py
+++ b/ct-unet_amd/ctunet_amd/ops.py
@@ -293,13 +293,20 @@
 
     def __post_init__(self):
         assert self.a.cp == self.b.cp and self.a.dims == self.b.dims and self.a.dtype == self.b.dtype
-        assert self.a.cp in (8, 16), "the two-segment head kernels take at most 16 channels per segment"
 
     @property
     def cp(self) -> int:
         return 2 * self.a.cp
 
     @property
+    def dtype(self) -> torch.dtype:
+        return self.a.dtype
+
+    @property
+    def nvox(self) -> int:
+        return self.a.nvox
+
+    @property
     def lp(self) -> int:
         return self.a.lp
 
@@ -309,6 +316,10 @@
 
     def seg_args(self):
         return self.a.ptr, self.a.cs, self.b.ptr, self.b.cs
+
+    def up_args(self):
+        assert self.a.cs == self.b.cs, "the two-segment up-convolution kernels take segments of equal voxel stride"
+        return self.a.ptr, self.b.ptr, self.a.cp, self.a.cs, self.cp
 
 
 def new_cl(n, d, h, w, cs, device, zero=False, dtype=torch.float32) -> torch.Tensor:
@@ -764,6 +775,7 @@
         out0 = torch.empty((n, 2, d, h, w_), dtype=torch.float32, device=dev)
         out1 = torch.empty((n, 2, d, h, w_), dtype=torch.float32, device=dev)
     seg2 = isinstance(x, CL2)
+    assert not seg2 or x.a.cp in (8, 16), "the two-segment head kernels take at most 16 channels per segment"
     src = (*x.seg_args(), x.a.cp) if seg2 else (x.ptr, x.cs, x.cp)
     _dual(x.lp, "head_fwd_seg2" if seg2 else "head_fwd", *src, _ptr(x.scale), _ptr(x.shift), int(x.relu), w.data_ptr(),
           b.data_ptr(), _ptr(imap), ci, co, act, head_mode, out0.data_ptr(), _ptr(out1), n, v, _stream())
@@ -782,6 +794,7 @@
     dev = w.device
     seg2 = isinstance(x, CL2)
     assert seg2 == isinstance(gin, CL2), "head_bwd: input and input gradient are both one buffer or both two segments"
+    assert not seg2 or x.a.cp in (8, 16), "the two-segment head kernels take at most 16 channels per segment"
     lib = _lib.load()
     ws = torch.empty(lib.ctu_head_bwd_ws_floats(n, v, x.cp, co), dtype=torch.float32, device=dev)
     dw = torch.empty_like(w)
@@ -922,6 +935,11 @@
     return bool(_lib.load().ctu_upconv_fused_supported(k, d, h, w, cin_p, nout_p))
 
 
+def upconv_fused_seg2_supported(dims, k: int, cin_p: int, nout_p: int, seg_c: int) -> bool:
+    n, d, h, w = dims
+    return bool(_lib.load().ctu_upconv_fused_seg2_supported(k, d, h, w, cin_p, nout_p, seg_c))
+
+
 def upconv_fused_pack(wt: torch.Tensor, bt: torch.Tensor, w3: torch.Tensor, cinv, cin_p: int, nout_p: int,
                       into=None):
     return _upconv_pack(wt, bt, w3, cinv, cin_p, nout_p, into, False)
@@ -958,7 +976,7 @@
     return _lib.load().ctu_upconv_fused_num_blocks(n, d, h, w, nout_p)
 
 
-def upconv_fused_fwd(x: CL, wp: torch.Tensor, beff: torch.Tensor, out: CL, stats: Optional[torch.Tensor],
+def upconv_fused_fwd(x, wp: torch.Tensor, beff: torch.Tensor, out: CL, stats: Optional[torch.Tensor],
                      algo_ch: Optional[Tuple[int, int]] = None, tail=None) -> None:
     n, d, h, w = x.dims
     assert out.dims == (n, 2 * d, 2 * h, 2 * w)
@@ -966,9 +984,11 @@
     vox = n * d * h * w
     with _timed(lambda: (f"upconv_fused_fwd_kernel<{out.cp}>", vox * (16.0 * ci * ci + 8 * 54.0 * ci * co),
                          4.0 * vox * (ci + 8 * co), (w, x.cp, out.cp))):
-        _lib.check(_lib.load().ctu_upconv_fused_fwd(x.ptr, x.cs, x.cp, _ptr(x.scale), _ptr(x.shift), int(x.relu),
-                                                    wp.data_ptr(), beff.data_ptr(), out.ptr, out.cs, out.cp, _ptr(stats),
-                                                    n, d, h, w, _tail_arg(tail), _stream()), "upconv_fused_fwd")
+        seg2 = isinstance(x, CL2)
+        entry = getattr(_lib.load(), "ctu_upconv_fused_fwd_seg2" if seg2 else "ctu_upconv_fused_fwd")
+        _lib.check(entry(*(x.up_args() if seg2 else (x.ptr, x.cs, x.cp)), _ptr(x.scale), _ptr(x.shift), int(x.relu),
+                         wp.data_ptr(), beff.data_ptr(), out.ptr, out.cs, out.cp, _ptr(stats),
+                         n, d, h, w, _tail_arg(tail), _stream()), "upconv_fused_fwd")
 
 
 def upconv_fused_wgrad_bn_supported(dims, cin_p: int, nout_p: int, dtype=torch.float32) -> bool:
@@ -976,20 +996,23 @@
     return dtype == torch.float32 and bool(_lib.load().ctu_upconv_fused_wgrad_bn_supported(n, d, h, w, cin_p, nout_p))
 
 
-def upconv_fused_wgrad(x: CL, g: CL, c: int, co: int, bt: torch.Tensor, pack_ws: torch.Tensor, imap, lazy=None):
+def upconv_fused_wgrad(x, g: CL, c: int, co: int, bt: torch.Tensor, pack_ws: torch.Tensor, imap, lazy=None):
     n, d, h, w = x.dims
     assert g.dims == (n, 2 * d, 2 * h, 2 * w) and not x.lp
     return _upconv_wgrad(x, g, c, co, bt, pack_ws, imap, lazy,
                          lambda: (f"upconv_fused_wgrad_kernel<{g.cp}> (+slab reduce)", 4.0 * (n * d * h * w) * (c + 8 * co)))
 
 
-def _upconv_wgrad(x: CL, g: CL, c: int, co: int, bt, pack_ws, imap, lazy, tag_bytes):
+def _upconv_wgrad(x, g: CL, c: int, co: int, bt, pack_ws, imap, lazy, tag_bytes):
     n, d, h, w = x.dims
-    dev = x.buf.device
+    dev = g.buf.device
+    seg2 = isinstance(x, CL2)
+    assert not (seg2 and x.lp)
+    sfx = "_seg2" if seg2 else ""
     gcp = () if x.lp else (g.cp,)
     dweff = torch.empty((8, 8, x.cp, g.cp), dtype=torch.float32, device=dev)
     ws = torch.empty(_query(x.lp, "upconv_fused_wgrad_ws_floats", n, d, h, w, x.cp, *gcp), dtype=torch.float32, device=dev)
-    act = (x.ptr, x.cs, x.cp, _ptr(x.scale), _ptr(x.shift), int(x.relu), g.ptr, g.cs, *gcp)
+    act = (*(x.up_args() if seg2 else (x.ptr, x.cs, x.cp)), _ptr(x.scale), _ptr(x.shift), int(x.relu), g.ptr, g.cs, *gcp)
     detail = (w, x.cp, g.cp)
 
     def record():
@@ -1000,11 +1023,11 @@
             y, vec, coef, gy = lazy
             assert y.dims == g.dims and gy.dims == g.dims and y.cs == g.cs == gy.cs and y.cp == g.cp == gy.cp
             assert gy.buf.data_ptr() != g.buf.data_ptr()
-            _dual(x.lp, "upconv_fused_wgrad_bn", *act, y.ptr, vec[0].data_ptr(), vec[1].data_ptr(), coef.data_ptr(), gy.ptr,
+            _dual(x.lp, "upconv_fused_wgrad_bn" + sfx, *act, y.ptr, vec[0].data_ptr(), vec[1].data_ptr(), coef.data_ptr(), gy.ptr,
                   dweff.data_ptr(), ws.data_ptr(), n, d, h, w, _stream())
             g = gy
         else:
-            _dual(x.lp, "upconv_fused_wgrad", *act, dweff.data_ptr(), ws.data_ptr(), n, d, h, w, _stream())
+            _dual(x.lp, "upconv_fused_wgrad" + sfx, *act, dweff.data_ptr(), ws.data_ptr(), n, d, h, w, _stream())
     dwt = torch.empty((c, c, 2, 2, 2), dtype=torch.float32, device=dev)
     dbt = torch.empty(c, dtype=torch.float32, device=dev)
     dw3 = torch.empty((co, c, 3, 3, 3), dtype=torch.float32, device=dev)
@@ -1077,15 +1100,17 @@
     return wpd
 
 
-def upconv_fused_bwd_data(g: CL, wpd: torch.Tensor, gin: CL, algo_ch: Optional[Tuple[int, int]] = None) -> None:
+def upconv_fused_bwd_data(g: CL, wpd: torch.Tensor, gin, algo_ch: Optional[Tuple[int, int]] = None) -> None:
     n, d, h, w = gin.dims
     assert g.dims == (n, 2 * d, 2 * h, 2 * w)
     ci, co = algo_ch if algo_ch is not None else (gin.cp, g.cp)
     vox = n * d * h * w
     with _timed(lambda: (f"upconv_fused_bwd_data_kernel<{g.cp}>", vox * (16.0 * ci * ci + 8 * 54.0 * ci * co),
                          4.0 * vox * (ci + 8 * co), (w, gin.cp, g.cp))):
-        _lib.check(_lib.load().ctu_upconv_fused_bwd_data(g.ptr, g.cs, g.cp, wpd.data_ptr(), gin.ptr, gin.cs, gin.cp,
-                                                         n, d, h, w, _stream()), "upconv_fused_bwd_data")
+        seg2 = isinstance(gin, CL2)
+        entry = getattr(_lib.load(), "ctu_upconv_fused_bwd_data_seg2" if seg2 else "ctu_upconv_fused_bwd_data")
+        _lib.check(entry(g.ptr, g.cs, g.cp, wpd.data_ptr(), *(gin.up_args() if seg2 else (gin.ptr, gin.cs, gin.cp)),
+                         n, d, h, w, _stream()), "upconv_fused_bwd_data")
 
 
 def _ncv(t: torch.Tensor):
diff --git a/include/ctunet_hip.h b/include/ctunet_hip.h
--- a/include/ctunet_hip.h
+++ b/include/ctunet_hip.h
@@ -267,6 +267,20 @@
 int ctu_upconv_fused_pack_bwd(const float* wp, int cin_p, int nout_p, float* wpd, void* stream);
 int ctu_upconv_fused_bwd_data(const float* gout, int g_cs, int nout_p, const float* wpd, float* gin, int gin_cs,
                               int cin_p, int N, int D, int H, int W, void* stream);
+
+int ctu_upconv_fused_seg2_supported(int k, int D, int H, int W, int cin_p, int nout_p, int seg_c);
+int ctu_upconv_fused_fwd_seg2(const float* in0, const float* in1, int seg_c, int cs, int cin_p, const float* in_scale,
+                              const float* in_shift, int in_relu, const float* wp, const float* beff, float* out, int out_cs,
+                              int nout_p, float* stats, int N, int D, int H, int W, const ctu_bn_tail* tail, void* stream);
+int ctu_upconv_fused_wgrad_seg2(const float* in0, const float* in1, int seg_c, int cs, int cin_p, const float* in_scale,
+                                const float* in_shift, int in_relu, const float* gout, int g_cs, int nout_p, float* dweff,
+                                float* ws, int N, int D, int H, int W, void* stream);
+int ctu_upconv_fused_wgrad_bn_seg2(const float* in0, const float* in1, int seg_c, int cs, int cin_p, const float* in_scale,
+                                   const float* in_shift, int in_relu, const float* ga, int g_cs, int nout_p, const float* y,
+                                   const float* bn_scale, const float* bn_shift, const float* coef, float* gy_out,
+                                   float* dweff, float* ws, int N, int D, int H, int W, void* stream);
+int ctu_upconv_fused_bwd_data_seg2(const float* gout, int g_cs, int nout_p, const float* wpd, float* gin0, float* gin1,
+                                   int seg_c, int cs, int cin_p, int N, int D, int H, int W, void* stream);
 
 int ctu_hard_segm(const float* prob, int N, int C, int64_t nvox_per_item, float* seg, void* stream);
 int ctu_one_hot(const float* label, int N, int C, int64_t nvox_per_item, float* out, void* stream);
```

New measurement: 722.0 million voxels/s (median of 6 runs). +1.3%, better.
